# apache/brpc

Measured on NVIDIA H100. Metric: echo QPS, 1 KB baidu_std, higher is better.
Workload: dtype u8

## Files before the change

### brpc_b200/abi.py

```python
import atexit
import ctypes as C
import gc
import os

import numpy as np

_HERE = os.path.dirname(os.path.abspath(__file__))
lib_path = os.environ.get("B2RPC_LIB") or os.path.join(_HERE, "libb2rpc.so")

B2_OK, B2_E_INVAL, B2_E_NO_DEVICE, B2_E_CUDA, B2_E_CAPACITY, B2_E_NOMEM = 0, -1, -2, -3, -4, -5

RUN_DT = np.dtype([("socket_id", "<u8"), ("offset", "<u4"), ("length", "<u4"),
                   ("preferred_proto", "<i4"), ("flags", "<u4")])
RUN_STATUS_DT = np.dtype([("consumed", "<u4"), ("parse_error", "<u4"), ("n_msgs", "<u4"), ("first_msg", "<u4"),
                          ("preferred_proto", "<i4"), ("n_unanswered", "<u4"), ("resp_off", "<u4"), ("resp_bytes", "<u4")])
H2_FRAME_DT = np.dtype([("type", "u1"), ("flags", "u1"), ("pad", "<u2"), ("stream_id", "<u4"), ("payload_off", "<u4"), ("payload_len", "<u4")])
HPACK_BLOCK_DT = np.dtype([("conn", "<u4"), ("offset", "<u4"), ("length", "<u4"), ("reserved", "<u4")])
H2_RUN_STATUS_DT = np.dtype([("consumed", "<u4"), ("parse_error", "<u4"), ("n_msgs", "<u4"), ("first_msg", "<u4"), ("ctrl_off", "<u4"), ("ctrl_len", "<u4"),
                             ("remote_max_frame_size", "<u4"), ("remote_stream_window_size", "<u4")])
REQUEST_DT = np.dtype([("kind", "<u4"), ("flags", "<u4"), ("method_idx", "<i4"), ("timeout_ms", "<i4"), ("correlation_id", "<i8"), ("log_id", "<i8"),
                       ("compress_type", "<i4"), ("checksum_type", "<i4"), ("frame_type", "<i4"), ("payload_off", "<u4"), ("payload_len", "<u4"),
                       ("attachment_off", "<u4"), ("attachment_len", "<u4"), ("reserved", "<u4")])
REPLY_DT = np.dtype([("flags", "<u4"), ("error_code", "<i4"), ("correlation_id", "<i8"), ("compress_type", "<i4"), ("checksum_type", "<i4"),
                     ("content_type", "<i4"), ("error_text_off", "<u4"), ("error_text_len", "<u4"), ("body_off", "<u4"), ("body_len", "<u4"),
                     ("attachment_off", "<u4"), ("attachment_len", "<u4"), ("checksum_value_off", "<u4"), ("checksum_value_len", "<u4"),
                     ("extra_streams_off", "<u4"), ("n_extra_streams", "<u4"), ("user_fields_off", "<u4"), ("n_user_fields", "<u4"),
                     ("reserved", "<u4"), ("stream_id", "<i8")])
H2_RESPONSE_DT = np.dtype([("conn", "<u4"), ("stream_id", "<u4"), ("status_code", "<i4"), ("flags", "<u4"), ("content_type_off", "<u4"),
                           ("content_type_len", "<u4"), ("body_off", "<u4"), ("body_len", "<u4"), ("grpc_status", "<i4"),
                           ("grpc_message_off", "<u4"), ("grpc_message_len", "<u4"), ("reserved", "<u4")])
H2_REQUEST_DT = np.dtype([("conn", "<u4"), ("flags", "<u4"), ("path_off", "<u4"), ("path_len", "<u4"), ("authority_off", "<u4"),
                          ("authority_len", "<u4"), ("content_type_off", "<u4"), ("content_type_len", "<u4"), ("body_off", "<u4"),
                          ("body_len", "<u4"), ("extra_off", "<u4"), ("extra_len", "<u4")])
H2_PEER_UPDATE_DT = np.dtype([("set", "<u4"), ("header_table_size", "<u4"), ("max_frame_size", "<u4"), ("stream_window_size", "<u4"), ("conn_window_add", "<i8")])
H2_REQUEST_RESULT_DT = np.dtype([("status", "<i4"), ("stream_id", "<u4"), ("out_off", "<u4"), ("out_len", "<u4")])
H2_MSG_DT = np.dtype([("run_idx", "<u4"), ("stream_id", "<u4"), ("headers_off", "<u4"), ("headers_len", "<u4"), ("n_headers", "<u4"),
                      ("body_off", "<u4"), ("body_len", "<u4"), ("http_method", "<u4"), ("content_type", "<u4"), ("flags", "<u4"),
                      ("method_idx", "<i4"), ("msg_off", "<u4"), ("msg_len", "<u4"), ("path_off", "<u4"), ("path_len", "<u4"), ("reserved", "<u4")])
H2_CALL_DT = np.dtype([("run_idx", "<u4"), ("stream_id", "<u4"), ("how", "<u4"), ("status_code", "<i4"), ("error_code", "<i4"), ("grpc_status", "<i4"),
                       ("headers_off", "<u4"), ("headers_len", "<u4"), ("n_headers", "<u4"), ("body_off", "<u4"), ("body_len", "<u4"),
                       ("msg_off", "<u4"), ("msg_len", "<u4"), ("error_off", "<u4"), ("error_len", "<u4"), ("flags", "<u4")])
H2_FLAG_GUNZIPPED, H2_FLAG_GUNZIP_HOST, H2_FLAG_NO_GRPC_ENCODING = 64, 128, 256
H2_FLAG_ANSWERED = 512
H2_REPLY_SPAN_DT = np.dtype([("off", "<u4"), ("len", "<u4"), ("n_answered", "<u4"), ("reserved", "<u4")])
MSG_DT = np.dtype([("run_idx", "<u4"), ("frame_off", "<u4"), ("body_size", "<u4"), ("meta_size", "<u4"),
                   ("correlation_id", "<i8"), ("log_id", "<i8"),
                   ("attachment_size", "<i4"), ("compress_type", "<i4"), ("checksum_type", "<i4"), ("error_code", "<i4"),
                   ("has_bits", "<u2"), ("protocol", "u1"), ("content_type", "u1"),
                   ("method_idx", "<i2"), ("status", "<u2"), ("resp_off", "<u4"), ("resp_len", "<u4")])
assert RUN_DT.itemsize == 24 and RUN_STATUS_DT.itemsize == 32 and MSG_DT.itemsize == 64
STREAM_DESC_DT = np.dtype([("stream_id", "<i8"), ("remote_stream_id", "<i8"), ("host_socket_id", "<u8"), ("flags", "<u4"), ("max_buf_size", "<u4")])
STREAM_MSG_DT = np.dtype([("stream_id", "<i8"), ("first_frame", "<u4"), ("n_frames", "<u4"), ("off", "<u4"), ("len", "<u4"), ("flags", "<u4"), ("reserved", "<u4")])
STREAM_EVENT_DT = np.dtype([("stream_id", "<i8"), ("host_socket_id", "<u8"), ("local_consumed", "<u8"), ("remote_consumed", "<u8"), ("n_msgs", "<u4"),
                            ("first_msg", "<u4"), ("consumed_bytes", "<u4"), ("flags", "<u4"), ("fb_off", "<u4"), ("fb_len", "<u4"), ("close_off", "<u4"),
                            ("close_len", "<u4"), ("handover_msg", "<u4"), ("pending_bytes", "<u4"), ("reserved", "<u4", (2,))])
assert STREAM_DESC_DT.itemsize == 32 and STREAM_MSG_DT.itemsize == 32 and STREAM_EVENT_DT.itemsize == 80
STREAM_CONNECTED, STREAM_NEED_FEEDBACK, STREAM_CLOSED, STREAM_HANDED_OVER = 1, 2, 4, 8
STREAM_MSG_IN_INPUT = 1
STREAM_EV_REMOTE_CONSUMED_MOVED, STREAM_EV_CLOSED_BY_RST, STREAM_EV_CLOSED_BY_CLOSE, STREAM_EV_HANDED_OVER, STREAM_EV_WRITABLE = 1, 2, 4, 8, 16
STREAM_WRITE_DT = np.dtype([("stream_id", "<i8"), ("flags", "<u4"), ("src_off", "<u4"), ("src_len", "<u4"), ("reserved", "<u4")])
STREAM_WRITE_RESULT_DT = np.dtype([("status", "<i4"), ("n_frames", "<u4"), ("out_off", "<u4"), ("out_len", "<u4"), ("produced", "<u8"),
                                   ("host_socket_id", "<u8")])
assert STREAM_WRITE_DT.itemsize == 24 and STREAM_WRITE_RESULT_DT.itemsize == 32
STREAM_W_FROM_MSG = 1
STREAM_W_NOT_CONNECTED, STREAM_W_HANDED_OVER = -1, -2
STREAM_W_DEFAULT_SEGMENT = 512 << 20


class Method(C.Structure):
    _fields_ = [("service_full_name", C.c_char_p), ("service_name", C.c_char_p), ("method_name", C.c_char_p),
                ("request_type_name", C.c_char_p), ("handler", C.c_int32), ("echo_attachment", C.c_int32),
                ("response_checksum_type", C.c_int32), ("response_compress_type", C.c_int32)]


class Options(C.Structure):
    _fields_ = [("device", C.c_int32), ("max_batch_bytes", C.c_uint32), ("max_msgs", C.c_uint32),
                ("max_runs", C.c_uint32), ("max_resp_bytes", C.c_uint32), ("tile_bytes", C.c_uint32),
                ("max_body_size", C.c_uint64)]


class BatchResult(C.Structure):
    _fields_ = [("runs", C.c_void_p), ("n_runs", C.c_uint32),
                ("msgs", C.c_void_p), ("n_msgs", C.c_uint32),
                ("resp", C.c_void_p), ("resp_bytes", C.c_uint32),
                ("kernel_ms", C.c_float), ("n_launches", C.c_uint32), ("refs", C.c_void_p), ("iov", C.c_void_p)]


class H2RingResult(C.Structure):
    _fields_ = [("runs", C.c_void_p), ("n_runs", C.c_uint32), ("n_msgs", C.c_uint32), ("msgs", C.c_void_p), ("out", C.c_void_p),
                ("region", C.c_uint32), ("replies", C.c_void_p), ("spans", C.c_void_p), ("status", C.c_int32)]


assert C.sizeof(H2RingResult) == 64


class H2ClientRingResult(C.Structure):
    _fields_ = [("runs", C.c_void_p), ("n_runs", C.c_uint32), ("n_calls", C.c_uint32), ("calls", C.c_void_p), ("out", C.c_void_p),
                ("region", C.c_uint32), ("n_reqs", C.c_uint32), ("reqs", C.c_void_p), ("req_out", C.c_void_p), ("status", C.c_int32),
                ("reserved", C.c_uint32)]


assert C.sizeof(H2ClientRingResult) == 64


class StreamState(C.Structure):
    _fields_ = [("local_consumed", C.c_uint64), ("remote_consumed", C.c_uint64), ("pending_bytes", C.c_uint32), ("flags", C.c_uint32),
                ("error_code", C.c_int32), ("reserved", C.c_uint32)]


class StreamBatchResult(C.Structure):
    _fields_ = [("msgs", C.c_void_p), ("n_msgs", C.c_uint32), ("events", C.c_void_p), ("n_events", C.c_uint32),
                ("out", C.c_void_p), ("out_bytes", C.c_uint32), ("ctrl", C.c_void_p), ("ctrl_bytes", C.c_uint32),
                ("run_ctrl", C.c_void_p), ("n_runs", C.c_uint32)]


REF_DT = np.dtype([("prefix_len", "<u4"), ("src_off", "<u4"), ("src_len", "<u4"), ("reserved", "<u4")])
IOVEC_DT = np.dtype([("base", "<u8"), ("len", "<u8")])
INPUT_COPY, INPUT_PULL, RESP_COPY, RESP_BY_REF, RESP_IOVEC = 0, 1, 0, 1, 2


class ResidentKernel(C.Structure):
    _fields_ = [("name", C.c_char_p), ("regs", C.c_uint32), ("threads", C.c_uint32), ("smem_bytes", C.c_uint32), ("fits", C.c_uint32)]


class B2Error(RuntimeError):
    def __init__(self, code, text):
        super().__init__("b2rpc error %d: %s" % (code, text))
        self.code = code


def _load():
    if not os.path.exists(lib_path):
        raise ImportError("brpc_b200/libb2rpc.so is missing: run `python -c 'import __graft_entry__ as g; g.build()'` "
                          "(nvcc, sm_90a).  There is no CPU fallback.")
    l = C.CDLL(lib_path)
    l.b2_last_error.restype = C.c_char_p
    l.b2_version.restype = C.c_char_p
    l.b2_ctx_create.argtypes = [C.POINTER(Options), C.POINTER(C.c_void_p)]
    l.b2_ctx_destroy.argtypes = [C.c_void_p]
    l.b2_register_method.argtypes = [C.c_void_p, C.POINTER(Method)]
    l.b2_set_server_identity.argtypes = [C.c_void_p, C.c_char_p]
    l.b2_set_stream_handler.argtypes = [C.c_void_p, C.c_int]
    l.b2_set_protocols.argtypes = [C.c_void_p, C.c_uint32]
    l.b2_block_alloc.restype = C.c_void_p; l.b2_block_alloc.argtypes = [C.c_size_t]
    l.b2_block_free.argtypes = [C.c_void_p]
    l.b2_block_pool_host_allocs.restype = C.c_uint64
    l.b2_set_modes.argtypes = [C.c_void_p, C.c_int, C.c_int]
    l.b2_ring_start.argtypes = [C.c_void_p]; l.b2_ring_stop.argtypes = [C.c_void_p]
    l.b2_ring_submit.argtypes = [C.c_void_p, C.c_void_p, C.c_uint32, C.c_void_p, C.c_uint32, C.POINTER(C.c_uint32)]
    l.b2_ring_wait.argtypes = [C.c_void_p, C.c_uint32, C.POINTER(BatchResult)]
    l.b2_ring_launches.restype = C.c_uint64; l.b2_ring_launches.argtypes = [C.c_void_p]
    l.b2_ring_phase_ns.argtypes = [C.c_void_p, C.c_uint32, C.c_void_p]
    l.b2_latency_probe.argtypes = [C.c_void_p, C.c_void_p, C.c_uint32, C.c_void_p, C.c_uint32, C.c_uint32, C.c_int, C.c_void_p]
    l.b2_process_batch.argtypes = [C.c_void_p, C.c_void_p, C.c_uint32, C.c_void_p, C.c_uint32, C.POINTER(BatchResult)]
    l.b2_batch_submit.argtypes = [C.c_void_p, C.c_void_p, C.c_uint32, C.c_void_p, C.c_uint32]
    l.b2_batch_collect.argtypes = [C.c_void_p, C.POINTER(BatchResult)]
    l.b2_batch_upload.argtypes = [C.c_void_p, C.c_void_p, C.c_uint32, C.c_void_p, C.c_uint32]
    l.b2_batch_execute.argtypes = [C.c_void_p, C.POINTER(C.c_float), C.POINTER(C.c_uint32)]
    l.b2_batch_execute_many.argtypes = [C.c_void_p, C.c_uint32, C.POINTER(C.c_float), C.POINTER(C.c_uint32)]
    l.b2_batch_launch.argtypes = [C.c_void_p]
    l.b2_batch_wait.argtypes = [C.c_void_p]
    l.b2_elapsed_ms.argtypes = [C.c_void_p, C.c_void_p, C.POINTER(C.c_float)]
    l.b2_batch_download.argtypes = [C.c_void_p, C.POINTER(BatchResult)]
    l.b2_batch_info.argtypes = [C.c_void_p, C.c_void_p]
    l.b2_resident_plan.argtypes = [C.c_void_p, C.POINTER(ResidentKernel), C.c_int]
    l.b2_device_pci_bus_id.argtypes = [C.c_int, C.c_char_p, C.c_int]
    l.b2_stage_times.argtypes = [C.c_void_p, C.POINTER(C.c_char_p), C.POINTER(C.c_float), C.c_int]
    l.b2_crc32c_batch.argtypes = [C.c_void_p, C.c_void_p, C.c_uint32, C.c_void_p, C.c_void_p, C.c_uint32, C.c_void_p]
    l.b2_snappy_uncompress_batch.argtypes = [C.c_void_p, C.c_void_p, C.c_uint32, C.c_void_p, C.c_void_p, C.c_uint32,
                                             C.c_void_p, C.c_uint32, C.c_void_p, C.c_void_p]
    l.b2_snappy_compress_batch.argtypes = [C.c_void_p, C.c_void_p, C.c_uint32, C.c_void_p, C.c_void_p, C.c_uint32,
                                           C.c_void_p, C.c_uint32, C.c_void_p, C.c_void_p]
    l.b2_crc32c_extend.restype = C.c_uint32; l.b2_crc32c_extend.argtypes = [C.c_uint32, C.c_char_p, C.c_size_t]
    l.b2_snappy_max_compressed_length.restype = C.c_size_t; l.b2_snappy_max_compressed_length.argtypes = [C.c_size_t]
    l.b2_snappy_raw_compress.argtypes = [C.c_char_p, C.c_size_t, C.c_void_p, C.POINTER(C.c_size_t)]
    l.b2_snappy_get_uncompressed_length.argtypes = [C.c_char_p, C.c_size_t, C.POINTER(C.c_size_t)]
    l.b2_snappy_raw_uncompress.argtypes = [C.c_char_p, C.c_size_t, C.c_void_p]
    l.b2_hpack_reset.argtypes = [C.c_void_p, C.c_uint32, C.c_uint32]
    l.b2_hpack_decode_batch.argtypes = [C.c_void_p, C.c_void_p, C.c_uint32, C.c_void_p, C.c_uint32, C.c_void_p, C.c_uint32,
                                        C.c_void_p, C.c_void_p, C.c_void_p]
    l.b2_h2_scan_batch.argtypes = [C.c_void_p, C.c_void_p, C.c_uint32, C.c_void_p, C.c_uint32, C.c_uint32, C.c_void_p, C.c_uint32,
                                   C.c_void_p, C.c_void_p, C.c_void_p]
    l.b2_h2_conn_reset.argtypes = [C.c_void_p, C.c_uint32]
    l.b2_h2_configure.argtypes = [C.c_void_p, C.c_uint32, C.c_uint32, C.c_uint32]
    l.b2_h2_process_batch.argtypes = [C.c_void_p, C.c_void_p, C.c_uint32, C.c_void_p, C.c_uint32, C.c_void_p, C.c_void_p, C.c_uint32,
                                      C.POINTER(C.c_uint32), C.c_void_p, C.c_uint32]
    l.b2_h2_pack_requests.argtypes = [C.c_void_p, C.c_void_p, C.c_uint32, C.c_void_p, C.c_uint32, C.c_void_p, C.c_uint32, C.c_void_p]
    l.b2_h2_conn_set_next_stream_id.argtypes = [C.c_void_p, C.c_uint32, C.c_uint32]
    l.b2_h2_conn_peer_update.argtypes = [C.c_void_p, C.c_uint32, C.c_void_p]
    l.b2_h2_client_conn_reset.argtypes = [C.c_void_p, C.c_uint32]
    l.b2_h2_client_process_batch.argtypes = [C.c_void_p, C.c_void_p, C.c_uint32, C.c_void_p, C.c_uint32, C.c_void_p, C.c_void_p, C.c_uint32,
                                             C.POINTER(C.c_uint32), C.c_void_p, C.c_uint32]
    l.b2_h2_client_abandon_streams.argtypes = [C.c_void_p, C.c_uint32, C.c_void_p, C.c_uint32]
    l.b2_h2_conn_set_gunzip.argtypes = [C.c_void_p, C.c_uint32, C.c_int]
    l.b2_h2_serve_batch.argtypes = [C.c_void_p, C.c_void_p, C.c_uint32, C.c_void_p, C.c_uint32, C.c_void_p, C.c_void_p, C.c_uint32,
                                    C.POINTER(C.c_uint32), C.c_void_p, C.c_uint32, C.c_void_p, C.c_uint32, C.c_void_p]
    l.b2_h2_ring_enable.argtypes = [C.c_void_p, C.c_uint32, C.c_uint32, C.c_uint32, C.c_uint32]
    l.b2_h2_ring_submit.argtypes = [C.c_void_p, C.c_void_p, C.c_uint32, C.c_void_p, C.c_uint32, C.POINTER(C.c_uint32)]
    l.b2_h2_ring_wait.argtypes = [C.c_void_p, C.c_uint32, C.POINTER(H2RingResult)]
    l.b2_h2_client_ring_enable.argtypes = [C.c_void_p, C.c_uint32, C.c_uint32, C.c_uint32, C.c_uint32, C.c_uint32]
    l.b2_h2_client_ring_submit.argtypes = [C.c_void_p, C.c_void_p, C.c_uint32, C.c_void_p, C.c_uint32, C.c_void_p, C.c_uint32, C.POINTER(C.c_uint32)]
    l.b2_h2_client_ring_wait.argtypes = [C.c_void_p, C.c_uint32, C.POINTER(H2ClientRingResult)]
    l.b2_h2_pack_responses.argtypes = [C.c_void_p, C.c_void_p, C.c_uint32, C.c_void_p, C.c_uint32, C.c_void_p, C.c_uint32, C.c_void_p, C.c_void_p]
    l.b2_pack_requests.argtypes = [C.c_void_p, C.c_void_p, C.c_uint32, C.c_void_p, C.c_uint32, C.c_void_p, C.c_uint32, C.c_void_p, C.c_void_p]
    l.b2_pack_responses.argtypes = [C.c_void_p, C.c_void_p, C.c_uint32, C.c_void_p, C.c_uint32, C.c_void_p, C.c_uint32, C.c_void_p, C.c_void_p]
    l.b2_stream_configure.argtypes = [C.c_void_p, C.c_uint32, C.c_uint32, C.c_uint32]
    l.b2_stream_open.argtypes = [C.c_void_p, C.c_void_p, C.c_uint32]
    l.b2_stream_set_connected.argtypes = [C.c_void_p, C.c_int64, C.c_int64, C.c_uint32, C.c_void_p, C.c_uint32, C.POINTER(C.c_uint32)]
    l.b2_stream_close.argtypes = [C.c_void_p, C.c_int64, C.c_void_p, C.c_uint32, C.POINTER(C.c_uint32)]
    l.b2_stream_query.argtypes = [C.c_void_p, C.c_int64, C.POINTER(StreamState)]
    l.b2_stream_take_pending.argtypes = [C.c_void_p, C.c_int64, C.c_void_p, C.c_uint32, C.POINTER(C.c_uint32)]
    l.b2_stream_results.argtypes = [C.c_void_p, C.POINTER(StreamBatchResult)]
    l.b2_stream_ring_enable.argtypes = [C.c_void_p, C.c_uint32]
    l.b2_stream_write.argtypes = [C.c_void_p, C.c_void_p, C.c_uint32, C.c_void_p, C.c_uint32, C.c_uint32, C.c_void_p, C.c_uint32, C.c_void_p]
    l.b2_counters_read.argtypes = [C.c_void_p, C.POINTER(C.c_int64)]
    l.b2_counters_device_ptr.restype = C.c_void_p; l.b2_counters_device_ptr.argtypes = [C.c_void_p]
    return l


lib = _load()

ABI_SYMBOLS = ["b2_ctx_create", "b2_ctx_destroy", "b2_last_error", "b2_version", "b2_register_method",
               "b2_set_server_identity", "b2_set_stream_handler", "b2_set_protocols", "b2_block_alloc", "b2_block_free", "b2_block_pool_host_allocs", "b2_set_modes", "b2_ring_start", "b2_ring_stop", "b2_ring_submit", "b2_ring_wait", "b2_ring_launches", "b2_ring_phase_ns", "b2_latency_probe", "b2_process_batch", "b2_batch_submit", "b2_batch_collect", "b2_batch_upload",
               "b2_batch_execute", "b2_batch_execute_many", "b2_batch_download", "b2_batch_launch", "b2_batch_wait",
               "b2_elapsed_ms", "b2_batch_info", "b2_resident_plan", "b2_device_pci_bus_id", "b2_stage_times", "b2_crc32c_batch", "b2_crc32c_extend", "b2_snappy_max_compressed_length", "b2_snappy_raw_compress", "b2_snappy_get_uncompressed_length", "b2_snappy_raw_uncompress", "b2_snappy_uncompress_batch", "b2_snappy_compress_batch", "b2_hpack_reset", "b2_hpack_decode_batch", "b2_pack_requests", "b2_pack_responses", "b2_h2_scan_batch", "b2_h2_conn_reset", "b2_h2_configure", "b2_h2_process_batch", "b2_h2_pack_responses", "b2_counters_read",
               "b2_counters_device_ptr", "b2_counters_allreduce", "b2_h2_pack_requests", "b2_h2_conn_set_next_stream_id", "b2_h2_conn_peer_update",
               "b2_h2_client_conn_reset", "b2_h2_client_process_batch", "b2_h2_client_abandon_streams", "b2_h2_conn_set_gunzip",
               "b2_h2_serve_batch", "b2_stream_configure", "b2_stream_open", "b2_stream_set_connected", "b2_stream_close", "b2_stream_query",
               "b2_stream_take_pending", "b2_stream_results", "b2_stream_write", "b2_stream_ring_enable", "b2_h2_ring_enable", "b2_h2_ring_submit",
               "b2_h2_ring_wait", "b2_h2_client_ring_enable", "b2_h2_client_ring_submit", "b2_h2_client_ring_wait"]

ECHO_METHOD = dict(service_full_name=b"example.EchoService", service_name=b"EchoService", method_name=b"Echo",
                   request_type_name=b"example.EchoRequest", handler=1, echo_attachment=1,
                   response_checksum_type=0, response_compress_type=0)


def _check(rc):
    if rc < 0:
        raise B2Error(rc, (lib.b2_last_error() or b"").decode("utf-8", "replace"))
    return rc


def _view(ptr, nbytes, dtype=np.uint8):
    return np.ctypeslib.as_array((C.c_uint8 * nbytes).from_address(ptr)).view(dtype) if nbytes else np.zeros(0, dtype)


_in_gc = [False]
_reclaimed = []


def _gc_phase(phase, info):
    _in_gc[0] = phase == "start"


def _destroy_reclaimed():
    hs = _reclaimed[:]
    del _reclaimed[:]
    for h in hs:
        lib.b2_ring_stop(h)
    for h in hs:
        lib.b2_ctx_destroy(h)


gc.callbacks.append(_gc_phase)
atexit.register(_destroy_reclaimed)


class PinnedBuffer:

    def __init__(self, nbytes):
        self.ptr = lib.b2_block_alloc(nbytes)
        if not self.ptr:
            raise B2Error(B2_E_NOMEM, "b2_block_alloc failed")
        self.nbytes = nbytes
        self.array = np.ctypeslib.as_array((C.c_uint8 * nbytes).from_address(self.ptr))

    def free(self):
        if self.ptr:
            lib.b2_block_free(self.ptr)
            self.ptr = None

    def __del__(self):
        try:
            self.free()
        except Exception:
            pass


class Context:

    def __init__(self, device=0, max_batch_bytes=64 << 20, max_msgs=1 << 20, max_runs=4096, max_resp_bytes=0,
                 tile_bytes=0, max_body_size=0, methods=(ECHO_METHOD,), server_identity=None, stream_handler=0):
        _destroy_reclaimed()
        opt = Options(device, max_batch_bytes, max_msgs, max_runs, max_resp_bytes, tile_bytes, max_body_size)
        h = C.c_void_p()
        _check(lib.b2_ctx_create(C.byref(opt), C.byref(h)))
        self._h = h
        self._keep = []
        for m in methods:
            self.register_method(**m)
        if server_identity:
            _check(lib.b2_set_server_identity(self._h, server_identity))
        if stream_handler:
            _check(lib.b2_set_stream_handler(self._h, stream_handler))

    def close(self):
        if getattr(self, "_h", None):
            lib.b2_ctx_destroy(self._h)
            self._h = None
        _destroy_reclaimed()

    def __del__(self):
        try:
            if _in_gc[0] and getattr(self, "_h", None):
                _reclaimed.append(self._h)
                self._h = None
            else:
                self.close()
        except Exception:
            pass

    def register_method(self, **kw):
        m = Method(**kw)
        self._keep.append(m)
        return _check(lib.b2_register_method(self._h, C.byref(m)))

    @staticmethod
    def _views(res):
        runs = np.ctypeslib.as_array((C.c_uint8 * (32 * res.n_runs)).from_address(res.runs)).view(RUN_STATUS_DT) \
            if res.n_runs else np.zeros(0, RUN_STATUS_DT)
        msgs = np.ctypeslib.as_array((C.c_uint8 * (64 * res.n_msgs)).from_address(res.msgs)).view(MSG_DT) \
            if res.n_msgs else np.zeros(0, MSG_DT)
        resp = np.ctypeslib.as_array((C.c_uint8 * res.resp_bytes).from_address(res.resp)) \
            if res.resp_bytes else np.zeros(0, np.uint8)
        return runs, msgs, resp

    @staticmethod
    def _info(res):
        refs = None
        if res.refs and res.n_msgs:
            refs = np.ctypeslib.as_array((C.c_uint8 * (16 * res.n_msgs)).from_address(res.refs)).view(REF_DT)
        iov = None
        if res.iov and res.n_msgs:
            iov = np.ctypeslib.as_array((C.c_uint8 * (32 * res.n_msgs)).from_address(res.iov)).view(IOVEC_DT)
        return {"kernel_ms": res.kernel_ms, "n_launches": res.n_launches, "refs": refs, "iov": iov}

    def _ring_bytes(self, data, ptr, nbytes):
        if ptr is None:
            data = np.ascontiguousarray(data, dtype=np.uint8); ptr, nbytes = data.ctypes.data, data.nbytes
            self._ring_keep = data
        return ptr, nbytes

    def ring_start(self):
        _check(lib.b2_ring_start(self._h))

    def ring_stop(self):
        _check(lib.b2_ring_stop(self._h))

    def ring_submit(self, data, runs, ptr=None, nbytes=None):
        runs = np.ascontiguousarray(runs, dtype=RUN_DT)
        ptr, nbytes = self._ring_bytes(data, ptr, nbytes)
        t = C.c_uint32(0)
        _check(lib.b2_ring_submit(self._h, ptr, nbytes, runs.ctypes.data, len(runs), C.byref(t)))
        return t.value

    def ring_wait(self, ticket):
        res = BatchResult()
        _check(lib.b2_ring_wait(self._h, ticket, C.byref(res)))
        rs, msgs, resp = self._views(res)
        return rs, msgs, resp, self._info(res)

    def latency_probe(self, ptr, nbytes, runs, iters, use_ring):
        runs = np.ascontiguousarray(runs, dtype=RUN_DT)
        us = np.zeros(iters, np.float32)
        _check(lib.b2_latency_probe(self._h, ptr, nbytes, runs.ctypes.data, len(runs), iters, 1 if use_ring else 0, us.ctypes.data))
        return us

    def ring_phase_ns(self, ticket):
        out = (C.c_uint64 * 4)()
        _check(lib.b2_ring_phase_ns(self._h, ticket, out))
        return list(out)

    def ring_launches(self):
        return int(lib.b2_ring_launches(self._h))

    def set_protocols(self, mask):
        _check(lib.b2_set_protocols(self._h, mask))

    def set_modes(self, input_mode=INPUT_COPY, resp_mode=RESP_COPY):
        _check(lib.b2_set_modes(self._h, input_mode, resp_mode))

    def process_batch(self, data, runs):
        data = np.ascontiguousarray(data, dtype=np.uint8)
        runs = np.ascontiguousarray(runs, dtype=RUN_DT)
        res = BatchResult()
        _check(lib.b2_process_batch(self._h, data.ctypes.data, data.nbytes, runs.ctypes.data, len(runs), C.byref(res)))
        rs, msgs, resp = self._views(res)
        return rs, msgs, resp, self._info(res)

    def upload(self, data, runs):
        data = np.ascontiguousarray(data, dtype=np.uint8)
        runs = np.ascontiguousarray(runs, dtype=RUN_DT)
        _check(lib.b2_batch_upload(self._h, data.ctypes.data, data.nbytes, runs.ctypes.data, len(runs)))

    def upload_ptr(self, ptr, nbytes, runs):
        runs = np.ascontiguousarray(runs, dtype=RUN_DT)
        _check(lib.b2_batch_upload(self._h, ptr, nbytes, runs.ctypes.data, len(runs)))

    def execute(self):
        ms, n = C.c_float(0), C.c_uint32(0)
        _check(lib.b2_batch_execute(self._h, C.byref(ms), C.byref(n)))
        return ms.value, n.value

    def execute_many(self, steps):
        ms, n = C.c_float(0), C.c_uint32(0)
        _check(lib.b2_batch_execute_many(self._h, steps, C.byref(ms), C.byref(n)))
        return ms.value, n.value

    def launch(self):
        _check(lib.b2_batch_launch(self._h))

    def wait(self):
        _check(lib.b2_batch_wait(self._h))

    def elapsed_ms_to(self, other):
        ms = C.c_float(0)
        _check(lib.b2_elapsed_ms(self._h, other._h, C.byref(ms)))
        return ms.value

    def download(self):
        res = BatchResult()
        _check(lib.b2_batch_download(self._h, C.byref(res)))
        rs, msgs, resp = self._views(res)
        return rs, msgs, resp, self._info(res)

    def process_batch_ptr(self, ptr, nbytes, runs):
        runs = np.ascontiguousarray(runs, dtype=RUN_DT)
        res = BatchResult()
        _check(lib.b2_process_batch(self._h, ptr, nbytes, runs.ctypes.data, len(runs), C.byref(res)))
        rs, msgs, resp = self._views(res)
        return rs, msgs, resp, self._info(res)

    def submit_ptr(self, ptr, nbytes, runs):
        runs = np.ascontiguousarray(runs, dtype=RUN_DT)
        self._submitted_runs = runs
        _check(lib.b2_batch_submit(self._h, ptr, nbytes, runs.ctypes.data, len(runs)))

    def collect(self):
        res = BatchResult()
        _check(lib.b2_batch_collect(self._h, C.byref(res)))
        rs, msgs, resp = self._views(res)
        return rs, msgs, resp, self._info(res)

    def stream_configure(self, max_streams, pending_bytes, out_bytes=0):
        _check(lib.b2_stream_configure(self._h, max_streams, pending_bytes, out_bytes))

    def stream_open(self, streams):
        if not isinstance(streams, np.ndarray):
            a = np.zeros(len(streams), STREAM_DESC_DT)
            for i, t in enumerate(streams):
                a[i] = tuple(t) + (0,) * (5 - len(t))
            streams = a
        streams = np.ascontiguousarray(streams, dtype=STREAM_DESC_DT)
        _check(lib.b2_stream_open(self._h, streams.ctypes.data, len(streams)))

    def stream_set_connected(self, stream_id, remote_stream_id, flags=0):
        buf = C.create_string_buffer(64); n = C.c_uint32(0)
        _check(lib.b2_stream_set_connected(self._h, stream_id, remote_stream_id, flags, buf, 64, C.byref(n)))
        return buf.raw[:n.value]

    def stream_close(self, stream_id):
        buf = C.create_string_buffer(64); n = C.c_uint32(0)
        _check(lib.b2_stream_close(self._h, stream_id, buf, 64, C.byref(n)))
        return buf.raw[:n.value]

    def stream_query(self, stream_id):
        st = StreamState()
        _check(lib.b2_stream_query(self._h, stream_id, C.byref(st)))
        return {"local_consumed": st.local_consumed, "remote_consumed": st.remote_consumed, "pending_bytes": st.pending_bytes,
                "flags": st.flags, "error_code": st.error_code}

    def stream_take_pending(self, stream_id, cap):
        buf = np.zeros(max(1, cap), np.uint8); n = C.c_uint32(0)
        _check(lib.b2_stream_take_pending(self._h, stream_id, buf.ctypes.data, cap, C.byref(n)))
        return buf[:n.value].tobytes()

    def stream_ring_enable(self, out_bytes):
        _check(lib.b2_stream_ring_enable(self._h, out_bytes))

    def stream_results(self):
        r = StreamBatchResult()
        _check(lib.b2_stream_results(self._h, C.byref(r)))
        return (_view(r.msgs, 32 * r.n_msgs, STREAM_MSG_DT), _view(r.events, 80 * r.n_events, STREAM_EVENT_DT), _view(r.out, r.out_bytes, np.uint8),
                _view(r.ctrl, r.ctrl_bytes, np.uint8), _view(r.run_ctrl, 8 * r.n_runs, np.uint32).reshape(-1, 2))

    def stream_write(self, writes, data=None, max_segment_size=0, out_cap=None, out=None):
        if not isinstance(writes, np.ndarray):
            a = np.zeros(len(writes), STREAM_WRITE_DT)
            for i, t in enumerate(writes):
                a[i] = tuple(t) + (0,) * (5 - len(t))
            writes = a
        writes = np.ascontiguousarray(writes, dtype=STREAM_WRITE_DT)
        n = len(writes)
        if data is None:
            ptr, nb = None, 0
        else:
            data = np.ascontiguousarray(np.frombuffer(data, np.uint8) if isinstance(data, (bytes, bytearray)) else data, dtype=np.uint8)
            ptr, nb = data.ctypes.data, data.nbytes
        if out is None:
            if out_cap is None:
                seg = max_segment_size or STREAM_W_DEFAULT_SEGMENT
                lens = np.where(writes["flags"] & STREAM_W_FROM_MSG, 0, writes["src_len"]).astype(np.int64)
                if np.any(writes["flags"] & STREAM_W_FROM_MSG):
                    sm = self.stream_results()[0]
                    fm = (writes["flags"] & STREAM_W_FROM_MSG) != 0
                    idx = writes["src_off"][fm].astype(np.int64)
                    lens[fm] = np.where(idx < len(sm), sm["len"][np.minimum(idx, max(len(sm) - 1, 0))] if len(sm) else 0, 0)
                nfr = np.maximum(1, (lens + seg - 1) // seg)
                out_cap = int(((lens + nfr * 38 + 15) // 16 * 16).sum())
            out = np.empty(max(1, out_cap), np.uint8)
        res = np.zeros(n, STREAM_WRITE_RESULT_DT)
        _check(lib.b2_stream_write(self._h, ptr, nb, writes.ctypes.data, n, max_segment_size, out.ctypes.data, out.nbytes, res.ctypes.data))
        return res, out

    def batch_info(self):
        out = (C.c_uint32 * 4)()
        _check(lib.b2_batch_info(self._h, out))
        return {"tile_bytes": out[0], "n_tiles": out[1], "spec_k": out[2], "fused": bool(out[3])}

    def resident_plan(self):
        out = (ResidentKernel * 8)()
        n = _check(lib.b2_resident_plan(self._h, out, 8))
        return [{"name": out[i].name.decode(), "regs": out[i].regs, "threads": out[i].threads, "smem_bytes": out[i].smem_bytes,
                 "fits": out[i].fits} for i in range(min(n, 8))]

    def stage_times(self):
        names = (C.c_char_p * 16)()
        ms = (C.c_float * 16)()
        n = lib.b2_stage_times(self._h, names, ms, 16)
        return [(names[i].decode(), ms[i]) for i in range(max(0, min(n, 16)))]
# ... 216 lines not shown
```

### brpc_b200/csrc/b2_api.cu

```cuda
#include <cuda_runtime.h>
#include <dlfcn.h>
#include <stdio.h>
#include <time.h>
#include <stdlib.h>
#include <string.h>
#include <algorithm>
#include <mutex>
#include <string>
#include <unordered_map>
#include <vector>
#include "b2_kernels.cuh"
#include "b2_h2.cuh"

using namespace b2;

static thread_local char g_err[512] = "";
static void set_err(const char* fmt, const char* a = "", const char* b = "") { snprintf(g_err, sizeof g_err, fmt, a, b); }

#define CU(call)                                                                          \
    do {                                                                                  \
        cudaError_t e_ = (call);                                                          \
        if (e_ != cudaSuccess) { set_err("%s: %s", #call, cudaGetErrorString(e_)); return B2_E_CUDA; } \
    } while (0)

namespace {
constexpr int kMaxStages = 16;
constexpr uint32_t kSmallBytes = 128 << 10;
constexpr uint32_t kSmallRuns = 512, kSmallMsgs = 1024;
constexpr size_t kSmallBlock = 64 + kSmallRuns * 32 + kSmallMsgs * (64 + 16) + (kSmallBytes + kSmallMsgs * 80 + 4096);
struct SmallLayout { uint32_t msgs, resp, off_rs, off_msgs, off_refs, off_resp, total; };
SmallLayout small_layout(uint32_t nbytes, uint32_t n_runs, uint32_t max_msgs) {
    const uint32_t mb = std::min(std::min(nbytes / 12 + 1, kSmallMsgs), max_msgs), resp = nbytes + mb * 80 + 2048, off_msgs = 64 + n_runs * 32;
    const uint32_t off_refs = off_msgs + mb * 64, off_resp = (off_refs + mb * 16 + 255u) & ~255u;
    return { mb, resp, 64, off_msgs, off_refs, off_resp, off_resp + resp };
}
constexpr uint32_t kSecEvents = 64, kSecMsgs = kSecEvents + kSmallMsgs * 80, kSecCtrl = kSecMsgs + kSmallMsgs * 32,
                   kSecRunCtrl = kSecCtrl + 3 * kStreamCtrlMax * kSmallMsgs, kSecOut = kSecRunCtrl + kSmallRuns * 8;
struct Stage { const char* name; cudaEvent_t ev; };
enum class RingKind { none, batch, batch_streams, h2_server, h2_client };
struct SlotLayout {
    uint64_t end = 256;
    uint32_t add(uint64_t bytes) { const uint64_t off = end; end = (end + bytes + 255u) & ~255ull; return (uint32_t)off; }
};
}

enum : int { kPlanFused, kPlanSearch, kPlanWalk, kPlanResolve, kPlanSlow, kPlanKernels };
struct b2_ctx {
    b2_options opt;
    DevConfig cfg;
    std::vector<DevMethod> methods;
    uint8_t* d_bytes = nullptr; b2_run* d_runs = nullptr; uint32_t* d_run_tile_base = nullptr;
    TileRec* d_tiles = nullptr; uint32_t* d_tile_base = nullptr; uint32_t* d_tile_scratch = nullptr; uint32_t* d_tile_spec = nullptr; b2_run_status* d_run_status = nullptr;
    uint32_t* d_frame_off = nullptr; uint32_t* d_frame_run = nullptr; b2_msg_desc* d_msgs = nullptr; MsgAux* d_aux = nullptr; PackJob* d_jobs = nullptr; uint32_t* d_slow_idx = nullptr; uint8_t* d_heads = nullptr;
    uint32_t* d_slot = nullptr; uint32_t* d_scan_tmp = nullptr; uint8_t* d_resp = nullptr; uint8_t* d_unz = nullptr; uint16_t* d_snappy_tab = nullptr; HpackState* d_hpack = nullptr; H2Conn* d_h2 = nullptr; H2Stream* d_h2_streams = nullptr; uint8_t* d_h2_slots = nullptr; uint32_t h2_max_conns = B2_H2_MAX_CONNS, h2_pending = B2_H2_MAX_PENDING, h2_stream_bytes = B2_H2_STREAM_BYTES; uint64_t h2_last_in = 0, h2_last_out = 0;
    uint32_t* d_frame_row = nullptr; uint4* d_rows = nullptr;
    std::vector<uint8_t> h2_gunzip; uint8_t* d_h2_gz_merge = nullptr;
    RingKind ring_kind = RingKind::none; RingDev ring_dev = {}; H2RingDev h2r_dev = {}; H2ClientRingDev h2c_dev = {};
    uint8_t* ring_slots = nullptr; volatile uint32_t* ring_ctl = nullptr; uint32_t* d_ring_ticket = nullptr; cudaStream_t ring_stream = nullptr;
    uint32_t ring_next = 1, ring_stride = 0; bool ring_collected[8] = { true, true, true, true, true, true, true, true };
    const void* ring_bytes[8] = {}; const void* ring_pin_base = nullptr; unsigned long long ring_pin_dev = 0; uint64_t ring_launches = 0;
    StreamPass sp_ring = {}; uint8_t* d_st_ring = nullptr; uint32_t ring_next_wait = 1, st_view_ticket = 0;
    uint32_t h2r_max_bytes = 0, h2r_msg_cap = 0, h2r_out_cap = 0, h2r_replies_cap = 0;
    uint32_t h2c_max_bytes = 0, h2c_call_cap = 0, h2c_out_cap = 0, h2c_max_reqs = 0, h2c_req_out_cap = 0;
    ulonglong2* d_iov = nullptr; b2_iovec* h_iov = nullptr; const void* host_bytes = nullptr;
    uint4* d_refs = nullptr; b2_resp_ref* h_refs = nullptr; int input_mode = B2_INPUT_COPY, resp_mode = B2_RESP_COPY; const uint8_t* pull_bytes = nullptr;
    uint32_t* d_crc_adv = nullptr; unsigned long long* d_counters = nullptr; uint32_t* d_totals = nullptr; DevMethod* d_methods = nullptr;
    size_t meta_tile_off = 0; uint32_t max_tiles = 0; uint32_t n_sms = 132; bool use_tma_pack = true; uint32_t stage_mask = 7;
    StreamPass sp = {}; bool has_streams = false, stream_armed = false, stream_ran = false, stream_valid = false;
    uint32_t st_max = 0, st_open = 0; std::vector<long long> st_keys; std::vector<uint8_t> st_state; std::vector<uint32_t> st_pool, st_pool_free;
    void* d_st_block[10] = {}; void* h_st_mapped[5] = {}; uint32_t* h_st_cnts = nullptr; uint8_t* h_st_out = nullptr; uint8_t* h_st_ctl = nullptr; uint8_t* d_st_ctl = nullptr;
    b2_stream_msg* h_st_msgs = nullptr; b2_stream_event* h_st_events = nullptr; uint8_t* h_st_ctrl = nullptr; uint32_t* h_st_run_ctrl = nullptr;
    cudaEvent_t st_ev[6] = {};
    const uint8_t* st_input = nullptr;
    void* d_sw[4] = {}; size_t sw_have[4] = {}; SwRec* h_sw_recs = nullptr; size_t h_sw_have = 0; uint32_t* h_sw_cnts = nullptr;
    cudaEvent_t sw_ev[8] = {}; bool sw_ran = false;
    b2_run_status* h_run_status = nullptr; b2_msg_desc* h_msgs = nullptr; uint8_t* h_resp = nullptr;
    uint32_t* h_totals = nullptr; uint32_t* h_run_tile_base = nullptr;
    uint32_t n_runs = 0, n_tiles = 0, nbytes = 0, max_run_tiles = 0; uint64_t covered = 0;
    bool uploaded = false, executed = false;
    cudaStream_t stream = nullptr;
    cudaEvent_t ev[kMaxStages + 1];
    const char* stage_names[kMaxStages];
    int n_stages = 0;
    float last_kernel_ms = 0.f; uint32_t last_launches = 0;
    cudaEvent_t ev_first = nullptr, ev_last = nullptr; bool first_pending = true;
    bool profile_stages = false; bool allow_small = true; bool use_fused = true; bool fused_last = false; bool slow_heavy = false;
    bool adaptive_tile = false; bool dense = false; uint32_t avg_frame = 0;
    uint8_t* d_meta = nullptr; uint8_t* h_meta = nullptr;
    uint8_t* d_small = nullptr; uint8_t* h_small = nullptr;
    bool small = false, small_copy_queued = false, use_fused_small = true; SmallLayout sm = {};
    b2_resident_kernel plan[kPlanKernels] = {}; uint32_t sm_regs = 0, sm_smem = 0, sm_warps = 0, sm_blocks = 0, block_smem_reserve = 0;
};

enum : unsigned { kDevInput = 1, kDevBatch = 2 };
static void overwrites(b2_ctx* c, unsigned what) {
    if (what & kDevInput) { c->h2_last_in = 0; c->h2_last_out = 0; if (c->st_input == c->d_bytes) c->st_input = nullptr; }
    if (what & kDevBatch) { c->uploaded = false; c->executed = false; }
}

static uint32_t g_crc_tab_host[256];
static void crc_table_init() {
    for (uint32_t i = 0; i < 256; i++) {
        uint32_t c = i;
        for (int k = 0; k < 8; k++) c = (c & 1) ? (c >> 1) ^ 0x82f63b78u : (c >> 1);
        g_crc_tab_host[i] = c;
    }
}

extern "C" const char* b2_last_error(void) { return g_err; }
extern "C" const char* b2_version(void) { return "brpc_b200 0.1 (sm_90a)"; }

namespace {
struct BlockPool {
    std::mutex mu;
    static constexpr size_t kSmall = 8192, kSlab = 4u << 20;
    std::vector<uint8_t*> slabs; std::vector<void*> small_free;
    std::unordered_map<void*, int> large_class;
    std::vector<void*> large_free[40];
    uint64_t n_host_alloc = 0;
    void* alloc(size_t size) {
        std::lock_guard<std::mutex> g(mu);
        if (size <= kSmall) {
            if (small_free.empty()) {
                uint8_t* slab = nullptr;
                if (cudaHostAlloc((void**)&slab, kSlab, cudaHostAllocMapped | cudaHostAllocPortable) != cudaSuccess) return nullptr;
                n_host_alloc++; slabs.push_back(slab);
                for (size_t o = 0; o + kSmall <= kSlab; o += kSmall) small_free.push_back(slab + o);
            }
            void* p = small_free.back(); small_free.pop_back(); return p;
        }
        int cls = 14; while (((size_t)1 << cls) < size) cls++;
        if (cls >= 40) return nullptr;
        if (!large_free[cls].empty()) { void* p = large_free[cls].back(); large_free[cls].pop_back(); return p; }
        void* p = nullptr;
        if (cudaHostAlloc(&p, ((size_t)1 << cls) + 1024, cudaHostAllocMapped | cudaHostAllocPortable) != cudaSuccess) return nullptr;
        n_host_alloc++; large_class[p] = cls;
        return p;
    }
    void free(void* p) {
        std::lock_guard<std::mutex> g(mu);
        auto it = large_class.find(p);
        if (it != large_class.end()) { large_free[it->second].push_back(p); return; }
        small_free.push_back(p);
    }
};
BlockPool& block_pool() { static BlockPool* p = new BlockPool; return *p; }
}
extern "C" void* b2_block_alloc(size_t size) {
    void* p = block_pool().alloc(size ? size : 1);
    if (!p) set_err("cudaHostAlloc failed");
    return p;
}
extern "C" void b2_block_free(void* p) { if (p) block_pool().free(p); }
extern "C" uint64_t b2_block_pool_host_allocs(void) { std::lock_guard<std::mutex> g(block_pool().mu); return block_pool().n_host_alloc; }

static void ring_halt(b2_ctx* c);
static void stream_free(b2_ctx* c);
static bool ring_busy(const b2_ctx* c) { for (uint32_t k = 0; k < kRingSlots; k++) if (!c->ring_collected[k]) return true; return false; }
static uint8_t* ring_slot(const b2_ctx* c, uint32_t ticket) { return c->ring_slots + (size_t)(ticket % kRingSlots) * c->ring_stride; }
static bool h2_ring_refuses(b2_ctx* c, bool writes_h2_state) {
    if (c->ring_kind != RingKind::h2_server && c->ring_kind != RingKind::h2_client) return false;
    if (ring_busy(c)) { set_err(c->ring_kind == RingKind::h2_server ? "an h2 ring ticket is outstanding: b2_h2_ring_wait it first" : "an h2 client ring ticket is outstanding: b2_h2_client_ring_wait it first"); return true; }
    if (writes_h2_state) ring_halt(c);
    return false;
}
extern "C" void b2_ctx_destroy(b2_ctx* c) {
    if (!c) return;
    cudaSetDevice(c->opt.device);
    ring_halt(c);
    if (c->ring_stream) cudaStreamDestroy(c->ring_stream);
    if (c->ring_slots) cudaFreeHost(c->ring_slots);
    if (c->ring_ctl) cudaFreeHost((void*)c->ring_ctl);
    cudaFree(c->d_ring_ticket);
    cudaFree(c->d_bytes); cudaFree(c->d_runs); cudaFree(c->d_run_tile_base); cudaFree(c->d_tiles); cudaFree(c->d_tile_base); cudaFree(c->d_tile_scratch); cudaFree(c->d_tile_spec);
    cudaFree(c->d_run_status); cudaFree(c->d_frame_off); cudaFree(c->d_frame_run); cudaFree(c->d_msgs); cudaFree(c->d_aux); cudaFree(c->d_jobs); cudaFree(c->d_slow_idx); cudaFree(c->d_heads); cudaFree(c->d_slot);
    cudaFree(c->d_scan_tmp); cudaFree(c->d_resp); cudaFree(c->d_unz); cudaFree(c->d_snappy_tab); cudaFree(c->d_refs); cudaFree(c->d_iov); cudaFreeHost(c->h_iov); cudaFree(c->d_frame_row); cudaFree(c->d_rows); cudaFreeHost(c->h_refs); cudaFree(c->d_hpack); cudaFree(c->d_h2); cudaFree(c->d_h2_streams); cudaFree(c->d_h2_slots); cudaFree(c->d_h2_gz_merge); cudaFree(c->d_counters); cudaFree(c->d_totals); cudaFree(c->d_methods); cudaFree(c->d_crc_adv); cudaFree(c->d_meta); cudaFree(c->d_small); cudaFreeHost(c->h_meta); cudaFreeHost(c->h_small);
    cudaFreeHost(c->h_run_status); cudaFreeHost(c->h_msgs); cudaFreeHost(c->h_resp); cudaFreeHost(c->h_totals);
    cudaFreeHost(c->h_run_tile_base);
    stream_free(c);
    for (int i = 0; i <= kMaxStages; i++) if (c->ev[i]) cudaEventDestroy(c->ev[i]);
    if (c->stream) cudaStreamDestroy(c->stream);
    delete c;
}

extern "C" int b2_ctx_create(const b2_options* o, b2_ctx** out) {
    if (!o || !out) { set_err("null argument"); return B2_E_INVAL; }
    int ndev = 0;
    if (cudaGetDeviceCount(&ndev) != cudaSuccess || ndev == 0) {
        set_err("no CUDA device: brpc_b200 has no CPU path"); return B2_E_NO_DEVICE;
    }
    if (o->device < 0 || o->device >= ndev) { set_err("bad device ordinal"); return B2_E_INVAL; }
    if (o->max_batch_bytes == 0 || o->max_batch_bytes >= (1u << 31) || o->max_msgs == 0 || o->max_runs == 0) {
        set_err("capacities must be non-zero and max_batch_bytes < 2 GiB"); return B2_E_INVAL;
    }
    CU(cudaSetDevice(o->device));
    b2_ctx* c = new b2_ctx();
    { int v = 132; cudaDeviceGetAttribute(&v, cudaDevAttrMultiProcessorCount, o->device); c->n_sms = (uint32_t)v; }
    for (int i = 0; i <= kMaxStages; i++) c->ev[i] = nullptr;
    c->opt = *o;
    c->adaptive_tile = o->tile_bytes == 0;
    uint32_t tile = o->tile_bytes ? o->tile_bytes : 8192;
    if (tile < 512 || (tile & (tile - 1))) { delete c; set_err("tile_bytes must be a power of two >= 512"); return B2_E_INVAL; }
    c->opt.tile_bytes = tile;
    if (c->opt.max_resp_bytes == 0) {
        uint64_t r = (uint64_t)o->max_batch_bytes + (uint64_t)o->max_msgs * 64 + (1u << 20);
        c->opt.max_resp_bytes = r > 0xfffffff0ull ? 0xfffffff0u : (uint32_t)r;
    }
    memset(&c->cfg, 0, sizeof c->cfg);
    c->cfg.max_body_size = o->max_body_size ? o->max_body_size : (64ull << 20);
    c->cfg.proto_mask = kProtoMaskDefault;
    c->cfg.tile_bytes = tile;
    c->cfg.tile_shift = 0; while ((1u << c->cfg.tile_shift) < tile) c->cfg.tile_shift++;
    c->max_tiles = o->max_batch_bytes / tile + o->max_runs + 1;
    const uint32_t scan_blocks = o->max_msgs / (kScanBlock * kScanItems) + 2;
#define ALLOC(ptr, bytes) do { if (cudaMalloc((void**)&(ptr), (bytes)) != cudaSuccess) { set_err("cudaMalloc %s failed", #ptr); b2_ctx_destroy(c); return B2_E_NOMEM; } } while (0)
#define HALLOC(ptr, bytes) do { if (cudaHostAlloc((void**)&(ptr), (bytes), cudaHostAllocDefault) != cudaSuccess) { set_err("cudaHostAlloc %s failed", #ptr); b2_ctx_destroy(c); return B2_E_NOMEM; } } while (0)
    ALLOC(c->d_bytes, (size_t)o->max_batch_bytes + 1024);
    ALLOC(c->d_runs, sizeof(b2_run) * (size_t)o->max_runs);
    ALLOC(c->d_run_tile_base, 4 * ((size_t)o->max_runs + 1));
    ALLOC(c->d_tiles, sizeof(TileRec) * (size_t)c->max_tiles);
    ALLOC(c->d_tile_base, 4 * (size_t)c->max_tiles);
    ALLOC(c->d_tile_scratch, 12 * (size_t)c->max_tiles);
    {
        size_t dense_tiles = (size_t)o->max_batch_bytes / 2048 + o->max_runs + 1; if (dense_tiles > c->max_tiles) dense_tiles = c->max_tiles;
        size_t words = (size_t)kSpecK * c->max_tiles; if ((size_t)kSpecKDense * dense_tiles > words) words = (size_t)kSpecKDense * dense_tiles;
        ALLOC(c->d_tile_spec, 4 * words);
    }
    ALLOC(c->d_run_status, sizeof(b2_run_status) * (size_t)o->max_runs);
    ALLOC(c->d_frame_off, 4 * (size_t)o->max_msgs);
    ALLOC(c->d_frame_run, 4 * (size_t)o->max_msgs);
    ALLOC(c->d_msgs, sizeof(b2_msg_desc) * (size_t)o->max_msgs);
    ALLOC(c->d_aux, sizeof(MsgAux) * (size_t)o->max_msgs);
    ALLOC(c->d_jobs, sizeof(PackJob) * (size_t)o->max_msgs);
    ALLOC(c->d_refs, sizeof(uint4) * (size_t)o->max_msgs);
    ALLOC(c->d_slow_idx, sizeof(uint32_t) * (size_t)o->max_msgs);
    ALLOC(c->d_heads, (size_t)kHeadBytes * (size_t)o->max_msgs);
    ALLOC(c->d_slot, 4 * ((size_t)o->max_msgs + 1));
    ALLOC(c->d_scan_tmp, 4 * (size_t)scan_blocks);
    ALLOC(c->d_resp, (size_t)c->opt.max_resp_bytes + 1024);
    ALLOC(c->d_unz, 2 * (size_t)c->opt.max_resp_bytes + 1024);
    ALLOC(c->d_snappy_tab, (size_t)kSnappyWarps * kSnappyMaxTable * 2);
    ALLOC(c->d_hpack, sizeof(HpackState) * (size_t)B2_HPACK_MAX_CONNS);
    CU(cudaMemset(c->d_hpack, 0, sizeof(HpackState) * (size_t)B2_HPACK_MAX_CONNS));
    ALLOC(c->d_counters, 8 * B2_N_COUNTERS);
    ALLOC(c->d_totals, 64);
    ALLOC(c->d_methods, sizeof(DevMethod) * 64);
    ALLOC(c->d_crc_adv, (kCrcHotWords + kCrcTreeWords) * 4);
    ALLOC(c->d_meta, (size_t)o->max_runs * 28 + 16 * (size_t)c->max_tiles + 64);
    ALLOC(c->d_small, kSmallBlock);
    HALLOC(c->h_meta, (size_t)o->max_runs * 28 + 16 * (size_t)c->max_tiles + 64);
    HALLOC(c->h_small, kSmallBlock);
    HALLOC(c->h_run_status, sizeof(b2_run_status) * (size_t)o->max_runs);
    HALLOC(c->h_msgs, sizeof(b2_msg_desc) * (size_t)o->max_msgs);
    HALLOC(c->h_refs, sizeof(b2_resp_ref) * (size_t)o->max_msgs);
    HALLOC(c->h_resp, (size_t)c->opt.max_resp_bytes);
    HALLOC(c->h_totals, 64);
    HALLOC(c->h_run_tile_base, 4 * ((size_t)o->max_runs + 1));
    CU(cudaMemset(c->d_counters, 0, 8 * B2_N_COUNTERS));
    CU(cudaMemset(c->d_bytes, 0, (size_t)o->max_batch_bytes + 1024));
    CU(cudaStreamCreateWithFlags(&c->stream, cudaStreamNonBlocking));
    for (int i = 0; i <= kMaxStages; i++) CU(cudaEventCreate(&c->ev[i]));
    CU(cudaEventCreate(&c->ev_first)); CU(cudaEventCreate(&c->ev_last));
    crc_table_init();
    CU(cudaMemcpyToSymbol(c_crc_table, g_crc_tab_host, sizeof g_crc_tab_host));
    {
        std::vector<uint32_t> tab(kCrcHotWords + kCrcTreeWords);
        auto adv = [&](uint32_t x, int bytes) { for (int k = 0; k < bytes; k++) x = g_crc_tab_host[x & 0xff] ^ (x >> 8); return x; };
        for (int k = 0; k < 16; k++) for (uint32_t b = 0; b < 256; b++) tab[k * 256 + b] = adv(g_crc_tab_host[b], k);
        for (int j = 0; j < 4; j++) for (uint32_t b = 0; b < 256; b++) tab[(16 + j) * 256 + b] = adv(b << (8 * j), 512);
        for (int t = 0; t < 5; t++) for (int j = 0; j < 4; j++) for (uint32_t b = 0; b < 256; b++)
            tab[kCrcHotWords + (t * 4 + j) * 256 + b] = adv(b << (8 * j), 16 << t);
        CU(cudaMemcpy(c->d_crc_adv, tab.data(), tab.size() * 4, cudaMemcpyHostToDevice));
    }
    CU(cudaFuncSetAttribute(k_resolve, cudaFuncAttributeMaxDynamicSharedMemorySize, 200 * 1024));
    CU(cudaFuncSetAttribute(k_pack_slow<false>, cudaFuncAttributeMaxDynamicSharedMemorySize, (int)(8 * kSnapRing)));
    CU(cudaFuncSetAttribute(k_pack_tma<kPackGroup>, cudaFuncAttributeMaxDynamicSharedMemorySize, (int)(sizeof(PackWarpSmem) * kPackWarps)));
    CU(cudaFuncSetAttribute(k_pack_tma<kPackGroupSmall>, cudaFuncAttributeMaxDynamicSharedMemorySize, (int)(sizeof(PackWarpSmem) * kPackWarps)));
    if (const char* e = getenv("B2_PACK")) c->use_tma_pack = strcmp(e, "reg") != 0;
    if (const char* e = getenv("B2_SMALL")) c->use_fused_small = strcmp(e, "off") != 0;
    if (const char* e = getenv("B2_FUSED")) c->use_fused = strcmp(e, "off") != 0;
    CU(cudaFuncSetAttribute(k_fused, cudaFuncAttributeMaxDynamicSharedMemorySize, (int)(sizeof(FusedWarpSmem) * (kFusedWarps > kFusedWarpsDense ? kFusedWarps : kFusedWarpsDense))));
    CU(cudaFuncSetAttribute(k_small, cudaFuncAttributeMaxDynamicSharedMemorySize, (int)sizeof(SmallSmem)));
#if defined(__NVCC__)
    {
        const void* fn[kPlanKernels] = { (const void*)k_fused, (const void*)k_tile_search, (const void*)k_tile_walk, (const void*)k_resolve, (const void*)k_pack_slow<true> };
        const char* name[kPlanKernels] = { "k_fused", "k_tile_search", "k_tile_walk", "k_resolve", "k_pack_slow<true>" };
        const uint32_t threads[kPlanKernels] = { 0, kSearchThreadsFused, 128, 256, kSlowLiteThreads };
        for (int k = 0; k < kPlanKernels; k++) {
            cudaFuncAttributes a;
            CU(cudaFuncGetAttributes(&a, fn[k]));
            c->plan[k].name = name[k]; c->plan[k].regs = (uint32_t)a.numRegs; c->plan[k].threads = threads[k]; c->plan[k].smem_bytes = (uint32_t)a.sharedSizeBytes;
        }
        int v[5] = {};
        CU(cudaDeviceGetAttribute(&v[0], cudaDevAttrMaxRegistersPerMultiprocessor, o->device));
        CU(cudaDeviceGetAttribute(&v[1], cudaDevAttrMaxSharedMemoryPerMultiprocessor, o->device));
        CU(cudaDeviceGetAttribute(&v[2], cudaDevAttrMaxThreadsPerMultiProcessor, o->device));
        CU(cudaDeviceGetAttribute(&v[3], cudaDevAttrMaxBlocksPerMultiprocessor, o->device));
        CU(cudaDeviceGetAttribute(&v[4], cudaDevAttrReservedSharedMemoryPerBlock, o->device));
        c->sm_regs = (uint32_t)v[0]; c->sm_smem = (uint32_t)v[1]; c->sm_warps = (uint32_t)v[2] / 32; c->sm_blocks = (uint32_t)v[3]; c->block_smem_reserve = (uint32_t)v[4];
    }
#endif
    *out = c;
    return B2_OK;
}

extern "C" int b2_set_server_identity(b2_ctx* c, const char* ip_port) {
    if (!c) return B2_E_INVAL;
    if (h2_ring_refuses(c, true)) return B2_E_INVAL;
    const size_t n = ip_port ? strlen(ip_port) : 0;
    if (n >= sizeof c->cfg.identity) { set_err("identity too long"); return B2_E_INVAL; }
    memset(c->cfg.identity, 0, sizeof c->cfg.identity);
    if (n) memcpy(c->cfg.identity, ip_port, n);
    c->cfg.identity_len = (uint32_t)n;
    return B2_OK;
}

extern "C" int b2_set_modes(b2_ctx* c, int input_mode, int resp_mode) {
    if (!c || (input_mode != B2_INPUT_COPY && input_mode != B2_INPUT_PULL) || (resp_mode != B2_RESP_COPY && resp_mode != B2_RESP_BY_REF && resp_mode != B2_RESP_IOVEC)) { set_err("bad mode"); return B2_E_INVAL; }
    static_assert(sizeof(b2_resp_ref) == sizeof(uint4), "b2_resp_ref is 16 bytes");
    static_assert(sizeof(b2_iovec) == sizeof(ulonglong2) && sizeof(void*) == 8, "b2_iovec is a 16-byte struct iovec");
    if (resp_mode == B2_RESP_IOVEC && !c->d_iov) {
        CU(cudaSetDevice(c->opt.device));
        if (cudaMalloc((void**)&c->d_iov, 32 * (size_t)c->opt.max_msgs) != cudaSuccess || cudaHostAlloc((void**)&c->h_iov, 32 * (size_t)c->opt.max_msgs, cudaHostAllocDefault) != cudaSuccess) {
            cudaFree(c->d_iov); c->d_iov = nullptr; cudaGetLastError(); set_err("allocation of the iovec list failed"); return B2_E_NOMEM;
        }
    }
    if (input_mode == B2_INPUT_PULL && !c->d_rows) {
        CU(cudaSetDevice(c->opt.device));
        const uint32_t tile = c->adaptive_tile ? 32768u : c->opt.tile_bytes;
        const size_t tiles = (size_t)c->opt.max_batch_bytes / tile + c->opt.max_runs + 1;
        const size_t rows = tiles * (tile >= 2048 ? kSpecKDense : kSpecK);
        if (cudaMalloc((void**)&c->d_rows, rows * 128) != cudaSuccess || cudaMalloc((void**)&c->d_frame_row, 4 * (size_t)c->opt.max_msgs) != cudaSuccess) {
            cudaFree(c->d_rows); c->d_rows = nullptr; cudaGetLastError(); set_err("cudaMalloc of the pull-mode row stash failed"); return B2_E_NOMEM;
        }
    }
    ring_halt(c);
    c->input_mode = input_mode; c->resp_mode = resp_mode; c->cfg.by_ref = resp_mode != B2_RESP_COPY; c->cfg.pull = input_mode == B2_INPUT_PULL; c->cfg.pull_vecs = resp_mode != B2_RESP_COPY ? 6u : 8u;
    overwrites(c, kDevBatch);
    return B2_OK;
}

extern "C" int b2_set_protocols(b2_ctx* c, uint32_t mask) {
    const uint32_t known = (1u << 1) | (1u << 2) | (1u << 3) | (1u << 4) | (1u << 12);
    if (!c || mask == 0 || (mask & ~known)) { set_err("unknown protocol in mask (baidu_std 1, streaming_rpc 2, hulu_pbrpc 3, sofa_pbrpc 4, nshead 12)"); return B2_E_INVAL; }
    ring_halt(c);
    c->cfg.proto_mask = mask;
    return B2_OK;
}

extern "C" int b2_set_stream_handler(b2_ctx* c, int kind) {
    if (!c || (kind != B2_STREAM_DESC_ONLY && kind != B2_STREAM_SNAPPY_UNCOMPRESS)) { set_err("bad stream handler"); return B2_E_INVAL; }
    c->cfg.stream_handler = (uint32_t)kind;
    return B2_OK;
}

extern "C" int b2_register_method(b2_ctx* c, const b2_method* m) {
    if (!c || !m || !m->service_full_name || !m->service_name || !m->method_name || !m->request_type_name) { set_err("null argument"); return B2_E_INVAL; }
    if (c->methods.size() >= 64) { set_err("method table full"); return B2_E_CAPACITY; }
    DevMethod d; memset(&d, 0, sizeof d);
    std::string full = std::string(m->service_full_name) + "." + m->method_name;
    if (full.size() >= sizeof d.full_method || strlen(m->service_name) >= sizeof d.service_short ||
        strlen(m->service_full_name) >= sizeof d.service_full || strlen(m->request_type_name) >= sizeof d.request_type) {
        set_err("method names too long"); return B2_E_INVAL;
    }
    memcpy(d.full_method, full.data(), full.size()); d.full_method_len = (uint32_t)full.size();
    d.service_short_len = (uint32_t)strlen(m->service_name); memcpy(d.service_short, m->service_name, d.service_short_len);
    d.service_full_len = (uint32_t)strlen(m->service_full_name); memcpy(d.service_full, m->service_full_name, d.service_full_len);
    d.request_type_len = (uint32_t)strlen(m->request_type_name); memcpy(d.request_type, m->request_type_name, d.request_type_len);
    d.handler = m->handler; d.echo_attachment = m->echo_attachment;
    d.response_checksum_type = m->response_checksum_type; d.response_compress_type = m->response_compress_type;
    ring_halt(c);
    c->methods.push_back(d);
    c->cfg.n_methods = (uint32_t)c->methods.size();
    CU(cudaSetDevice(c->opt.device));
    CU(cudaMemcpy(c->d_methods, c->methods.data(), sizeof(DevMethod) * c->methods.size(), cudaMemcpyHostToDevice));
    return (int)c->methods.size() - 1;
}

static BatchPtrs make_ptrs(b2_ctx* c) {
    BatchPtrs B;
    B.bytes = c->d_bytes; B.runs = c->d_runs; B.run_tile_base = c->d_run_tile_base; B.tiles = c->d_tiles;
    B.tile_base = c->d_tile_base; B.tile_scratch = c->d_tile_scratch; B.tile_spec = c->d_tile_spec; B.run_status = c->d_run_status; B.frame_off = c->d_frame_off; B.frame_run = c->d_frame_run; B.frame_row = c->d_frame_row; B.rows = c->d_rows; B.msgs = c->d_msgs;
    B.aux = c->d_aux; B.jobs = c->d_jobs; B.refs = c->d_refs; B.slow_idx = c->d_slow_idx; B.heads = c->d_heads; B.slot = c->d_slot; B.scan_tmp = c->d_scan_tmp; B.resp = c->d_resp; B.unz = c->d_unz; B.snappy_tab = c->d_snappy_tab; B.counters = c->d_counters;
    B.totals = c->d_totals; B.methods = c->d_methods; B.crc_adv = c->d_crc_adv;
    B.n_runs = c->n_runs; B.n_tiles = c->n_tiles; B.max_msgs = c->opt.max_msgs; B.max_resp = c->opt.max_resp_bytes;
    B.runs = reinterpret_cast<const b2_run*>(c->d_meta);
    B.run_tile_base = reinterpret_cast<const uint32_t*>(c->d_meta + (size_t)c->n_runs * sizeof(b2_run));
    B.tile_info = reinterpret_cast<const uint4*>(c->d_meta + c->meta_tile_off);
    if (c->input_mode == B2_INPUT_PULL) B.bytes = c->pull_bytes;
    if (c->small) {
        B.refs = reinterpret_cast<uint4*>(c->d_small + c->sm.off_refs);
        B.totals = reinterpret_cast<uint32_t*>(c->d_small);
        B.run_status = reinterpret_cast<b2_run_status*>(c->d_small + c->sm.off_rs);
        B.msgs = reinterpret_cast<b2_msg_desc*>(c->d_small + c->sm.off_msgs);
        B.resp = c->d_small + c->sm.off_resp;
        B.max_msgs = c->sm.msgs; B.max_resp = c->sm.resp;
    }
    return B;
}

extern "C" int b2_batch_upload(b2_ctx* c, const void* bytes, uint32_t nbytes, const b2_run* runs, uint32_t n_runs) {
    if (!c || (!bytes && nbytes) || (!runs && n_runs)) { set_err("null argument"); return B2_E_INVAL; }
    if (h2_ring_refuses(c, false)) return B2_E_INVAL;
    if ((c->input_mode != B2_INPUT_PULL && nbytes > c->opt.max_batch_bytes) || nbytes >= (1u << 31) || n_runs > c->opt.max_runs) { set_err("batch exceeds ctx capacity"); return B2_E_CAPACITY; }
    uint64_t covered = 0; for (uint32_t r = 0; r < n_runs; r++) covered += runs[r].length;
    if (c->input_mode == B2_INPUT_PULL && covered > c->opt.max_batch_bytes) { set_err("runs exceed ctx capacity"); return B2_E_CAPACITY; }
    c->stream_valid = false; c->st_view_ticket = 0;
    c->covered = covered;
    CU(cudaSetDevice(c->opt.device));
    if (!c->avg_frame && n_runs && runs[0].length >= 12 && (uint64_t)runs[0].offset + 12 <= nbytes) {
        const uint8_t* f = static_cast<const uint8_t*>(bytes) + runs[0].offset;
        uint32_t w[2]; memcpy(w, f, 8);
        const uint32_t body = __builtin_bswap32(w[1]);
        if ((w[0] == kMagicPRPC || w[0] == kMagicSTRM) && body <= c->cfg.max_body_size && body < (1u << 30)) c->avg_frame = 12 + body;
    }
    if (c->adaptive_tile) {
        uint32_t t = 8192;
        const uint32_t per_tile = c->input_mode == B2_INPUT_PULL ? 48u : 6u;
        if (c->input_mode == B2_INPUT_PULL && t < 32768) t = 32768;
        while (t < (1u << 20) && t < per_tile * c->avg_frame) t <<= 1;
        c->cfg.tile_bytes = t; c->cfg.tile_shift = 0; while ((1u << c->cfg.tile_shift) < t) c->cfg.tile_shift++;
    }
    const uint32_t shift = c->cfg.tile_shift, tile = c->cfg.tile_bytes;
    c->dense = tile >= 2048 && c->avg_frame && (uint64_t)c->avg_frame * kSpecK < tile;
    c->cfg.spec_k = c->dense ? kSpecKDense : kSpecK;
    uint64_t nt = 0; uint32_t max_rt = 0;
    for (uint32_t r = 0; r < n_runs; r++) {
        if ((runs[r].offset & 15u) || (uint64_t)runs[r].offset + runs[r].length > nbytes) { set_err("run offset must be 16-aligned and inside the batch"); return B2_E_INVAL; }
        c->h_run_tile_base[r] = (uint32_t)nt;
        const uint32_t t = (uint32_t)(((uint64_t)runs[r].length + tile - 1) >> shift);
        nt += t; if (t > max_rt) max_rt = t;
    }
    c->h_run_tile_base[n_runs] = (uint32_t)nt;
    if (nt > c->max_tiles) { set_err("too many tiles"); return B2_E_CAPACITY; }
    c->n_runs = n_runs; c->n_tiles = (uint32_t)nt; c->nbytes = nbytes; c->max_run_tiles = max_rt; c->host_bytes = bytes;
    const size_t tile_off = ((size_t)n_runs * sizeof(b2_run) + 4 * ((size_t)n_runs + 1) + 15) & ~(size_t)15;
    const size_t meta_bytes = tile_off + 16 * (size_t)nt;
    c->meta_tile_off = tile_off;
    if (n_runs) memcpy(c->h_meta, runs, (size_t)n_runs * sizeof(b2_run));
    memcpy(c->h_meta + (size_t)n_runs * sizeof(b2_run), c->h_run_tile_base, 4 * ((size_t)n_runs + 1));
    {
        uint32_t* ti = reinterpret_cast<uint32_t*>(c->h_meta + tile_off);
        for (uint32_t r = 0; r < n_runs; r++) {
            const uint32_t t0 = c->h_run_tile_base[r], t1 = c->h_run_tile_base[r + 1];
            for (uint32_t t = t0; t < t1; t++) { uint32_t* q = ti + 4 * (size_t)t; q[0] = runs[r].offset; q[1] = runs[r].length; q[2] = t - t0; q[3] = r | (runs[r].flags << 24); }
        }
    }
    overwrites(c, kDevInput | kDevBatch);
    if (c->input_mode == B2_INPUT_PULL) {
        void* dp = nullptr;
        if (nbytes && cudaHostGetDevicePointer(&dp, const_cast<void*>(bytes), 0) != cudaSuccess) {
            cudaGetLastError(); set_err("B2_INPUT_PULL: bytes must be pinned + mapped memory from b2_block_alloc"); return B2_E_INVAL;
        }
        c->pull_bytes = static_cast<const uint8_t*>(dp);
    } else if (nbytes) CU(cudaMemcpyAsync(c->d_bytes, bytes, nbytes, cudaMemcpyHostToDevice, c->stream));
    CU(cudaMemcpyAsync(c->d_meta, c->h_meta, meta_bytes, cudaMemcpyHostToDevice, c->stream));
    c->small = c->allow_small && nbytes <= kSmallBytes && n_runs <= kSmallRuns && n_runs > 0;
    if (c->small) c->sm = small_layout(nbytes, n_runs, c->opt.max_msgs);
    if (const char* e = getenv("B2_STAGE_MASK")) c->stage_mask = (uint32_t)atoi(e);
    c->uploaded = true;
    return B2_OK;
}

static const char* const kStreamStages[5] = { "stream_route", "stream_alloc", "stream_group", "stream_run", "stream_rst" };
static uint32_t grid(uint32_t items, uint32_t per_block, uint32_t most) { const uint32_t g = (items + per_block - 1) / per_block; return g < 1 ? 1u : g < most ? g : most; }
static int launch_stream_pass(b2_ctx* c, const BatchPtrs& B, cudaStream_t s, uint32_t& launches) {
    const StreamPass& S = c->sp;
    const uint32_t msg_bound = c->small ? c->sm.msgs : c->opt.max_msgs, sms = c->n_sms;
    CU(cudaMemsetAsync(S.cnts, 0, 4 * (16 + 2 * (size_t)S.cap), s));
    CU(cudaEventRecord(c->st_ev[0], s));
    k_stream_route<<<grid(msg_bound, 256, sms * 4), 256, 0, s>>>(B, S); CU(cudaEventRecord(c->st_ev[1], s));
    k_stream_alloc<<<grid(c->st_max, 256, sms), 256, 0, s>>>(B, S); CU(cudaEventRecord(c->st_ev[2], s));
    k_stream_group<<<grid(msg_bound, 256, sms * 4), 256, 0, s>>>(B, S); CU(cudaEventRecord(c->st_ev[3], s));
    k_stream_run<<<grid(c->st_max, 4, sms * 8), 128, 0, s>>>(B, S); CU(cudaEventRecord(c->st_ev[4], s));
    k_stream_rst<<<grid(c->n_runs, 4, sms * 4), 128, 0, s>>>(B, S); CU(cudaEventRecord(c->st_ev[5], s));
    CU(cudaMemcpyAsync(c->h_st_cnts, S.cnts, 64, cudaMemcpyDeviceToHost, s));
    if (c->ring_kind == RingKind::batch_streams) CU(cudaMemsetAsync(S.cnt, 0, 8 * (size_t)S.cap, s));
    launches += 5; c->stream_ran = true; c->st_input = B.bytes;
    return B2_OK;
}

static uint32_t fused_warps(const b2_ctx* c) { return c->avg_frame && !c->dense ? kFusedWarps : kFusedWarpsDense; }
static size_t resolve_smem(const b2_ctx* c, bool fused) { const size_t b = (size_t)c->max_run_tiles * 12; return fused || b > 200 * 1024 ? 0 : b; }

static int launch_pipeline(b2_ctx* c, bool timed = true) {
    const BatchPtrs B = make_ptrs(c);
    DevConfig C = c->cfg;
    const bool fused = c->use_fused && !c->slow_heavy && !c->small && c->input_mode == B2_INPUT_COPY && c->resp_mode == B2_RESP_COPY && c->use_tma_pack &&
                       (((uint64_t)c->nbytes + 255) & ~255ull) + 4096 <= c->opt.max_resp_bytes;
    C.fused = fused ? 1u : 0u; C.ovf_base = (c->nbytes + 255u) & ~255u; c->fused_last = fused;
    cudaStream_t s = c->stream;
    int st = 0; uint32_t launches = 0;
    const bool prof = c->profile_stages;
    auto mark = [&](const char* name) { if (prof) { c->stage_names[st] = name; cudaEventRecord(c->ev[st + 1], s); st++; } };
    const uint32_t mask = c->stage_mask;
    const bool small_launch = c->small && c->use_fused_small && !prof;
    const bool search_zeroes = (mask & 1) && c->n_runs && c->n_tiles && !small_launch;
    if ((mask & 1) && !search_zeroes) CU(cudaMemsetAsync(B.totals, 0, 48, s));
    if (timed) CU(cudaEventRecord(c->ev[0], s));
    c->stream_ran = false;
    if (c->n_runs == 0) { c->n_stages = 0; c->last_launches = 0; return B2_OK; }
    if (small_launch) {
        k_small<<<1, kSmallThreads, sizeof(SmallSmem), s>>>(B, C);
        launches = 1;
        if (c->stream_armed) { int rc = launch_stream_pass(c, B, s, launches); if (rc != B2_OK) return rc; }
        c->stage_names[0] = "fused_small";
        if (timed) cudaEventRecord(c->ev[1], s);
        c->n_stages = timed ? 1 : 0; c->last_launches = launches;
        CU(cudaGetLastError());
        return B2_OK;
    }
    const uint32_t sms = c->n_sms;
    if (mask & 1) {
    if (c->n_tiles) {
        const uint32_t search_threads = fused ? kSearchThreadsFused : 256u;
        k_tile_search<<<(c->n_tiles * 32 + search_threads - 1) / search_threads, search_threads, 0, s>>>(B, C); launches++; mark("tile_search");
        if (C.pull) k_tile_walk_pull<<<(uint32_t)(((uint64_t)c->n_tiles * 8 + 127) / 128), 128, 0, s>>>(B, C);
        else k_tile_walk<<<(c->n_tiles + 127) / 128, 128, 0, s>>>(B, C);
        launches++; mark("tile_walk");
    }
    {
        const size_t smem = resolve_smem(c, fused);
        k_resolve<<<c->n_runs, 256, smem, s>>>(B, C, smem == 0 ? 1u : 0u); launches++; mark("resolve");
    }
    if (fused) {
        const uint32_t fw = fused_warps(c);
        if (c->n_tiles) { k_fused<<<sms, fw * 32, sizeof(FusedWarpSmem) * fw, s>>>(B, C); launches++; mark("fused"); }
    } else {
    if (c->n_tiles) { k_frame_table<<<(uint32_t)(((uint64_t)c->n_tiles * C.spec_k + 255) / 256), 256, 0, s>>>(B, C); launches++; mark("frame_table"); }
    k_decode<<<sms * B2_DECODE_MIN_BLOCKS, kDecodeWarps * 32, 0, s>>>(B, C); launches++; mark("decode");
    k_scan_blocks<<<sms, kScanBlock, 0, s>>>(B); launches++;
    mark("scan");
    }
    }
    if (fused) {
        if (mask & 4) { k_pack_slow<true><<<sms * B2_SLOW_MIN_BLOCKS * (256 / kSlowLiteThreads), kSlowLiteThreads, 0, s>>>(B, C); launches++; mark("pack_slow"); }
    } else if (c->use_tma_pack) {
        if (mask & 4) {
            if (c->slow_heavy || c->cfg.by_ref) { C.verify_done = 1; k_crc_verify<<<sms * 6, 256, 0, s>>>(B, C); launches++; mark("crc_verify"); }
            k_pack_slow<false><<<sms * B2_SLOW_MIN_BLOCKS, 256, 8 * kSnapRing, s>>>(B, C); launches++; mark("pack_slow");
        }
        if (mask & 2) {
            if ((c->avg_frame && c->avg_frame < 640) || c->cfg.by_ref) k_pack_tma<kPackGroupSmall><<<sms, kPackWarps * 32, sizeof(PackWarpSmem) * kPackWarps, s>>>(B, C);
            else k_pack_tma<kPackGroup><<<sms, kPackWarps * 32, sizeof(PackWarpSmem) * kPackWarps, s>>>(B, C);
            launches++; mark("pack");
        }
    } else { k_pack<<<sms * B2_PACK_MIN_BLOCKS, 256, 0, s>>>(B, C); launches++; mark("pack"); }
    if (c->resp_mode == B2_RESP_IOVEC && !c->small) {
        k_emit_iov<<<sms * 4, 256, 0, s>>>(B, c->d_iov, (unsigned long long)(uintptr_t)c->h_resp, (unsigned long long)(uintptr_t)c->host_bytes);
        launches++; mark("emit_iov");
    }
    if (c->stream_armed) { int rc = launch_stream_pass(c, B, s, launches); if (rc != B2_OK) return rc; }
    if (!prof && timed) { c->stage_names[0] = "pipeline"; cudaEventRecord(c->ev[1], s); st = 1; }
    c->n_stages = st; c->last_launches = launches;
    CU(cudaGetLastError());
    return B2_OK;
}

static bool replay_refused(const b2_ctx* c) {
    if (!c || !c->uploaded) { set_err("no batch uploaded"); return true; }
    if (c->stream_armed) { set_err("a submitted batch of a context with a stream table must be collected first: this entry point replays a batch and does not run the stream pass"); return true; }
    return false;
}
extern "C" int b2_batch_execute(b2_ctx* c, float* kernel_ms, uint32_t* n_launches) {
    if (replay_refused(c)) return B2_E_INVAL;
    CU(cudaSetDevice(c->opt.device));
    c->profile_stages = true;
    int rc = launch_pipeline(c);
    c->profile_stages = false;
    if (rc != B2_OK) return rc;
    CU(cudaStreamSynchronize(c->stream));
    float ms = 0.f;
    if (c->n_stages) CU(cudaEventElapsedTime(&ms, c->ev[0], c->ev[c->n_stages]));
    c->last_kernel_ms = ms; c->executed = true;
    if (kernel_ms) *kernel_ms = ms;
    if (n_launches) *n_launches = c->last_launches;
    return B2_OK;
}

extern "C" int b2_batch_execute_many(b2_ctx* c, uint32_t steps, float* total_ms, uint32_t* n_launches) {
    if (steps == 0) { set_err("no batch uploaded"); return B2_E_INVAL; }
    if (replay_refused(c)) return B2_E_INVAL;
    CU(cudaSetDevice(c->opt.device));
    cudaEvent_t e0, e1;
    CU(cudaEventCreate(&e0)); CU(cudaEventCreate(&e1));
    CU(cudaEventRecord(e0, c->stream));
    uint32_t launches = 0;
    for (uint32_t i = 0; i < steps; i++) {
        int rc = launch_pipeline(c);
        if (rc != B2_OK) return rc;
        launches += c->last_launches;
    }
    CU(cudaEventRecord(e1, c->stream));
    CU(cudaStreamSynchronize(c->stream));
    float ms = 0.f;
    CU(cudaEventElapsedTime(&ms, e0, e1));
    cudaEventDestroy(e0); cudaEventDestroy(e1);
    c->executed = true;
    if (c->n_stages) { float t = 0.f; cudaEventElapsedTime(&t, c->ev[0], c->ev[c->n_stages]); c->last_kernel_ms = t; }
    if (total_ms) *total_ms = ms;
    if (n_launches) *n_launches = launches;
    return B2_OK;
}

extern "C" int b2_batch_launch(b2_ctx* c) {
    if (replay_refused(c)) return B2_E_INVAL;
    CU(cudaSetDevice(c->opt.device));
    if (c->first_pending) { CU(cudaEventRecord(c->ev_first, c->stream)); c->first_pending = false; }
    int rc = launch_pipeline(c, false);
    if (rc != B2_OK) return rc;
    CU(cudaEventRecord(c->ev_last, c->stream));
    c->executed = true;
    return B2_OK;
}
extern "C" int b2_batch_wait(b2_ctx* c) {
    if (!c) return B2_E_INVAL;
    CU(cudaSetDevice(c->opt.device));
    CU(cudaStreamSynchronize(c->stream));
    c->first_pending = true;
    return B2_OK;
}
extern "C" int b2_elapsed_ms(b2_ctx* a, b2_ctx* b, float* ms) {
    if (!a || !b || !ms) return B2_E_INVAL;
    CU(cudaSetDevice(a->opt.device));
    CU(cudaEventElapsedTime(ms, a->ev_first, b->ev_last));
    return B2_OK;
}

static void refs_to_iov(b2_ctx* c, b2_batch_result* out, const void* host_bytes) {
    b2_run_status* rs = const_cast<b2_run_status*>(out->runs);
    for (uint32_t r = 0; r < out->n_runs; r++) rs[r].n_unanswered = 0;
    for (uint32_t i = 0; i < out->n_msgs; i++) {
        const b2_msg_desc& d = out->msgs[i];
        b2_iovec a = { const_cast<uint8_t*>(out->resp), 0 }, b = a;
        if (d.status == B2_MSG_ECHOED || d.status == B2_MSG_ERROR_REPLIED) {
            const b2_resp_ref rf = d.status == B2_MSG_ECHOED ? out->refs[i] : b2_resp_ref{0, 0, 0, 0};
            a.iov_base = const_cast<uint8_t*>(out->resp) + d.resp_off; a.iov_len = rf.src_len ? rf.prefix_len : d.resp_len;
            if (rf.src_len) { b.iov_base = const_cast<uint8_t*>(static_cast<const uint8_t*>(host_bytes)) + rf.src_off; b.iov_len = rf.src_len; }
        } else rs[d.run_idx].n_unanswered++;
        c->h_iov[2 * (size_t)i] = a; c->h_iov[2 * (size_t)i + 1] = b;
    }
    out->iov = c->h_iov; out->refs = nullptr;
}

static int download_normal(b2_ctx* c, b2_batch_result* out) {
    CU(cudaMemcpyAsync(c->h_totals, c->d_totals, 48, cudaMemcpyDeviceToHost, c->stream));
    CU(cudaStreamSynchronize(c->stream));
    if (c->n_runs && c->fused_last) {
        const bool heavy = (uint64_t)c->h_totals[3] * 8 > c->h_totals[0];
        if ((c->h_totals[2] & 2u) && !(c->h_totals[2] & 1u)) {
            c->slow_heavy = true;
            int rc = launch_pipeline(c); if (rc != B2_OK) return rc;
            CU(cudaMemcpyAsync(c->h_totals, c->d_totals, 48, cudaMemcpyDeviceToHost, c->stream));
            CU(cudaStreamSynchronize(c->stream));
        }
        c->slow_heavy = heavy || c->slow_heavy;
    } else if (c->n_runs && c->slow_heavy && !c->small) {
        c->slow_heavy = ((uint64_t)c->h_totals[3] + c->h_totals[7]) * 8 > c->h_totals[0];
    }
    if (c->n_runs && (c->h_totals[2] & 3u)) {
        set_err(c->h_totals[2] & 1u ? "more messages than max_msgs" : "responses exceed max_resp_bytes"); return B2_E_CAPACITY;
    }
    if (c->n_runs && c->fused_last) c->h_totals[1] = ((c->nbytes + 255u) & ~255u) + c->h_totals[9];
    const uint32_t n_msgs = c->n_runs ? c->h_totals[0] : 0, resp_bytes = c->n_runs ? c->h_totals[1] : 0;
    if (c->n_runs) CU(cudaMemcpyAsync(c->h_run_status, c->d_run_status, sizeof(b2_run_status) * c->n_runs, cudaMemcpyDeviceToHost, c->stream));
    if (n_msgs) CU(cudaMemcpyAsync(c->h_msgs, c->d_msgs, sizeof(b2_msg_desc) * (size_t)n_msgs, cudaMemcpyDeviceToHost, c->stream));
    if (resp_bytes) CU(cudaMemcpyAsync(c->h_resp, c->d_resp, resp_bytes, cudaMemcpyDeviceToHost, c->stream));
    const bool iovec = c->resp_mode == B2_RESP_IOVEC;
    if (n_msgs && c->cfg.by_ref && !iovec) CU(cudaMemcpyAsync(c->h_refs, c->d_refs, sizeof(b2_resp_ref) * (size_t)n_msgs, cudaMemcpyDeviceToHost, c->stream));
    if (n_msgs && iovec) CU(cudaMemcpyAsync(c->h_iov, c->d_iov, 32 * (size_t)n_msgs, cudaMemcpyDeviceToHost, c->stream));
// ... 438 lines not shown
    else {
        cudaPointerAttributes at; memset(&at, 0, sizeof at);
        if (cudaPointerGetAttributes(&at, bytes) == cudaSuccess && at.type == cudaMemoryTypeHost && at.devicePointer) {
            dev = (unsigned long long)(uintptr_t)at.devicePointer; c->ring_pin_base = bytes; c->ring_pin_dev = dev;
        } else cudaGetLastError();
    }
    if (!dev) { memcpy(slot + c->ring_dev.off_in, bytes, nbytes); dev = (unsigned long long)(uintptr_t)(slot + c->ring_dev.off_in); }
    return dev;
}
static uint8_t* ring_claim(b2_ctx* c, const char* wait_call) {
    if (!c->ring_collected[c->ring_next % kRingSlots]) { set_err("submit ring full: %s the oldest ticket first", wait_call); return nullptr; }
    return ring_slot(c, c->ring_next);
}
static RingSlotHdr* ring_fill(b2_ctx* c, uint8_t* slot, const void* bytes, uint32_t nbytes, const b2_run* runs, uint32_t n_runs) {
    overwrites(c, kDevInput | kDevBatch);
    RingSlotHdr* h = reinterpret_cast<RingSlotHdr*>(slot);
    h->bytes_dev = ring_stage(c, slot, bytes, nbytes);
    if (n_runs) memcpy(slot + c->ring_dev.off_runs, runs, sizeof(b2_run) * (size_t)n_runs);
    h->n_runs = n_runs; h->nbytes = nbytes;
    return h;
}
static int ring_ring(b2_ctx* c, RingSlotHdr* h, const void* bytes, uint32_t* ticket) {
    const uint32_t t = c->ring_next;
    c->ring_bytes[t % kRingSlots] = bytes; c->ring_collected[t % kRingSlots] = false;
    __sync_synchronize();
    h->submit = t;
    __sync_synchronize();
    c->ring_next = t + 1;
    *ticket = t;
    if (!c->ring_ctl[1]) { CU(cudaSetDevice(c->opt.device)); return ring_launch(c); }
    return B2_OK;
}
static int ring_spin(b2_ctx* c, const RingSlotHdr* h, uint32_t ticket) {
    uint64_t spins = 0;
    while (h->done != ticket) {
#if defined(__x86_64__)
        __builtin_ia32_pause();
#endif
        if ((++spins & 0xfffff) == 0) {
            if (!c->ring_ctl[1]) { CU(cudaSetDevice(c->opt.device)); int rc = ring_launch(c); if (rc != B2_OK) return rc; }
            if (cudaStreamQuery(c->ring_stream) != cudaErrorNotReady && h->done != ticket && !c->ring_ctl[1]) continue;
            if (spins > (1ull << 34)) { set_err("ring kernel did not answer"); return B2_E_CUDA; }
        }
    }
    __sync_synchronize();
    return B2_OK;
}
static uint8_t* ring_collect(b2_ctx* c, bool args_ok, uint32_t ticket, const char* bad_ticket, int& rc) {
    rc = B2_E_INVAL;
    if (!args_ok || !c->ring_slots || ticket == 0 || ticket >= c->ring_next || ticket + kRingSlots < c->ring_next) { set_err(bad_ticket); return nullptr; }
    if (c->ring_collected[ticket % kRingSlots]) { set_err("ticket already collected"); return nullptr; }
    const bool in_order = c->ring_kind == RingKind::batch_streams;
    if (in_order && ticket != c->ring_next_wait) { set_err("a context whose ring runs the stream pass collects its tickets in ticket order"); return nullptr; }
    uint8_t* slot = ring_slot(c, ticket);
    if ((rc = ring_spin(c, reinterpret_cast<const RingSlotHdr*>(slot), ticket)) != B2_OK) return nullptr;
    c->ring_collected[ticket % kRingSlots] = true;
    if (in_order) c->ring_next_wait = ticket + 1;
    return slot;
}
extern "C" int b2_ring_stop(b2_ctx* c) { if (!c) return B2_E_INVAL; cudaSetDevice(c->opt.device); ring_halt(c); return B2_OK; }

extern "C" int b2_ring_submit(b2_ctx* c, const void* bytes, uint32_t nbytes, const b2_run* runs, uint32_t n_runs, uint32_t* ticket) {
    if (!c || !bytes || !runs || !ticket || n_runs == 0) { set_err("null argument"); return B2_E_INVAL; }
    if (c->has_streams && c->ring_kind != RingKind::batch_streams) { set_err("the ring path runs the stream pass only after b2_stream_ring_enable: use b2_batch_submit on a context with a stream table"); return B2_E_INVAL; }
    if (c->ring_kind == RingKind::h2_server) { set_err("this context's ring serves h2 (b2_h2_ring_enable): use b2_h2_ring_submit"); return B2_E_INVAL; }
    if (c->ring_kind == RingKind::h2_client) { set_err("this context's ring serves h2 client connections (b2_h2_client_ring_enable): use b2_h2_client_ring_submit"); return B2_E_INVAL; }
    if (nbytes > kSmallBytes || n_runs > kSmallRuns) { set_err("b2_ring_submit serves batches up to 128 KiB / 512 runs: use b2_batch_submit"); return B2_E_CAPACITY; }
    if (!c->ring_slots) { int rc = b2_ring_start(c); if (rc != B2_OK) return rc; }
    uint8_t* slot = ring_claim(c, "b2_ring_wait");
    if (!slot) return B2_E_CAPACITY;
    for (uint32_t r = 0; r < n_runs; r++)
        if ((runs[r].offset & 15u) || (uint64_t)runs[r].offset + runs[r].length > nbytes) { set_err("run offset must be 16-aligned and inside the batch"); return B2_E_INVAL; }
    RingSlotHdr* h = ring_fill(c, slot, bytes, nbytes, runs, n_runs);
    const SmallLayout L = small_layout(nbytes, n_runs, c->opt.max_msgs);
    h->small_msgs = L.msgs; h->small_resp = L.resp; h->off_rs = L.off_rs; h->off_msgs = L.off_msgs;
    h->off_refs = L.off_refs; h->off_resp = L.off_resp; h->total = L.total; h->by_ref = c->cfg.by_ref;
    return ring_ring(c, h, bytes, ticket);
}

extern "C" int b2_ring_wait(b2_ctx* c, uint32_t ticket, b2_batch_result* out) {
    if (c && c->ring_kind == RingKind::h2_server) { set_err("this context's ring serves h2: use b2_h2_ring_wait"); return B2_E_INVAL; }
    if (c && c->ring_kind == RingKind::h2_client) { set_err("this context's ring serves h2 client connections: use b2_h2_client_ring_wait"); return B2_E_INVAL; }
    int rc;
    uint8_t* slot = ring_collect(c, c && out, ticket, "bad ring ticket", rc);
    if (!slot) return rc;
    const uint32_t si = ticket % kRingSlots;
    const bool streams = c->ring_kind == RingKind::batch_streams;
    RingSlotHdr* h = reinterpret_cast<RingSlotHdr*>(slot);
    memset(out, 0, sizeof *out);
    const uint8_t* ob = slot + c->ring_dev.off_out;
    const uint32_t* tot = reinterpret_cast<const uint32_t*>(ob);
    if (tot[2] & 3u) {
        if (!streams && ring_busy(c)) { set_err("ring overflow fallback needs the other tickets collected first"); return B2_E_CAPACITY; }
        if (!streams) ring_halt(c);
        const bool allow = c->allow_small; c->allow_small = false;
        rc = b2_process_batch(c, c->ring_bytes[si], h->nbytes, reinterpret_cast<const b2_run*>(slot + c->ring_dev.off_runs), h->n_runs, out);
        c->allow_small = allow;
        if (streams) { __sync_synchronize(); c->ring_ctl[3] = ticket; __sync_synchronize(); }
        return rc;
    }
    out->runs = reinterpret_cast<const b2_run_status*>(ob + h->off_rs); out->n_runs = h->n_runs;
    out->msgs = reinterpret_cast<const b2_msg_desc*>(ob + h->off_msgs); out->n_msgs = tot[0];
    out->resp = ob + h->off_resp; out->resp_bytes = tot[1];
    out->refs = h->by_ref ? reinterpret_cast<const b2_resp_ref*>(ob + h->off_refs) : nullptr;
    if (c->resp_mode == B2_RESP_IOVEC) refs_to_iov(c, out, c->ring_bytes[si]);
    out->n_launches = 0; out->kernel_ms = 0.f;
    if (streams) { c->stream_valid = true; c->st_view_ticket = ticket; c->st_input = c->d_bytes; }
    note_avg_frame(c, h->nbytes, out->n_msgs);
    return B2_OK;
}
extern "C" uint64_t b2_ring_launches(b2_ctx* c) { return c ? c->ring_launches : 0; }
extern "C" int b2_ring_phase_ns(b2_ctx* c, uint32_t ticket, uint64_t out[4]) {
    if (!c || !c->ring_slots || !out) return B2_E_INVAL;
    const RingSlotHdr* h = reinterpret_cast<const RingSlotHdr*>(ring_slot(c, ticket));
    for (int k = 0; k < 4; k++) out[k] = h->stamps[k + 1] - h->stamps[0];
    return B2_OK;
}

extern "C" int b2_latency_probe(b2_ctx* c, const void* bytes, uint32_t nbytes, const b2_run* runs, uint32_t n_runs, uint32_t iters, int use_ring, float* us_out) {
    if (!c || !us_out) return B2_E_INVAL;
    b2_batch_result res;
    for (uint32_t i = 0; i < iters; i++) {
        timespec t0, t1; clock_gettime(CLOCK_MONOTONIC, &t0);
        int rc;
        if (use_ring) { uint32_t t = 0; rc = b2_ring_submit(c, bytes, nbytes, runs, n_runs, &t); if (rc == B2_OK) rc = b2_ring_wait(c, t, &res); }
        else rc = b2_process_batch(c, bytes, nbytes, runs, n_runs, &res);
        clock_gettime(CLOCK_MONOTONIC, &t1);
        if (rc != B2_OK) return rc;
        if (res.n_msgs == 0) { set_err("latency probe batch produced no messages"); return B2_E_INVAL; }
        us_out[i] = (float)((t1.tv_sec - t0.tv_sec) * 1e6 + (t1.tv_nsec - t0.tv_nsec) * 1e-3);
    }
    return B2_OK;
}

extern "C" int b2_stage_times(b2_ctx* c, const char** names, float* ms, int cap) {
    if (!c) return B2_E_INVAL;
    int n = c->n_stages < cap ? c->n_stages : cap;
    for (int i = 0; i < n; i++) {
        names[i] = c->stage_names[i];
        float t = 0.f;
        cudaEventElapsedTime(&t, c->ev[i], c->ev[i + 1]);
        ms[i] = t;
    }
    int total = c->n_stages;
    if (c->stream_valid && c->stream_ran) {
        for (int i = 0; i < 5; i++, total++) if (total < cap) { names[total] = kStreamStages[i]; float t = 0.f; cudaEventElapsedTime(&t, c->st_ev[i], c->st_ev[i + 1]); ms[total] = t; }
    }
    if (c->sw_ran) {
        for (int i = 0; i < 7; i++, total++) if (total < cap) { names[total] = kSwStages[i]; float t = 0.f; cudaEventElapsedTime(&t, c->sw_ev[i], c->sw_ev[i + 1]); ms[total] = t; }
    }
    return total;
}

extern "C" int b2_batch_info(b2_ctx* c, uint32_t out[4]) {
    if (!c || !out) return B2_E_INVAL;
    out[0] = c->cfg.tile_bytes; out[1] = c->n_tiles; out[2] = c->cfg.spec_k; out[3] = c->fused_last ? 1u : 0u;
    return B2_OK;
}

static uint32_t block_regs(const b2_resident_kernel& k) { return (k.threads + 31) / 32 * ((k.regs * 32 + 255) / 256 * 256); }
static uint32_t smem_step(uint32_t bytes, uint32_t most) {
    static const uint32_t kKB[] = { 0, 8, 16, 32, 64, 100, 132, 164, 196, 228 };
    for (uint32_t kb : kKB) if (kb * 1024 >= bytes) return std::min(kb * 1024, most);
    return most;
}
extern "C" int b2_resident_plan(b2_ctx* c, b2_resident_kernel* out, int cap) {
    if (!c || (!out && cap > 0)) { set_err("null argument"); return B2_E_INVAL; }
    if (!c->plan[kPlanFused].name) { set_err("this build has no function attributes to plan with"); return B2_E_INVAL; }
    b2_resident_kernel k[kPlanKernels];
    memcpy(k, c->plan, sizeof k);
    const uint32_t fw = fused_warps(c);
    k[kPlanFused].threads = fw * 32; k[kPlanFused].smem_bytes += (uint32_t)(sizeof(FusedWarpSmem) * fw);
    k[kPlanResolve].smem_bytes += (uint32_t)resolve_smem(c, true);
    const b2_resident_kernel& f = k[kPlanFused];
    const uint32_t f_regs = block_regs(f), f_smem = f.smem_bytes + c->block_smem_reserve;
    const uint32_t room_regs = c->sm_regs > f_regs ? c->sm_regs - f_regs : 0, f_step = smem_step(f_smem, c->sm_smem);
    const uint32_t room_smem = f_step > f_smem ? f_step - f_smem : 0;
    const uint32_t room_warps = c->sm_warps > fw ? c->sm_warps - fw : 0, room_blocks = c->sm_blocks > 1 ? c->sm_blocks - 1 : 0;
    for (int i = 0; i < kPlanKernels; i++) {
        uint32_t n = room_blocks;
        n = std::min(n, room_regs / std::max(1u, block_regs(k[i])));
        n = std::min(n, room_smem / (k[i].smem_bytes + c->block_smem_reserve));
        n = std::min(n, room_warps / ((k[i].threads + 31) / 32));
        k[i].fits = n;
    }
    for (int i = 0; i < kPlanKernels && i < cap; i++) out[i] = k[i];
    return kPlanKernels;
}

extern "C" int b2_device_pci_bus_id(int device, char* out, int cap) {
    if (!out || cap < 13) return B2_E_INVAL;
    if (cudaDeviceGetPCIBusId(out, cap, device) != cudaSuccess) { cudaGetLastError(); return B2_E_CUDA; }
    return B2_OK;
}

extern "C" int b2_counters_read(b2_ctx* c, int64_t out[B2_N_COUNTERS]) {
    if (!c || !out) return B2_E_INVAL;
    CU(cudaSetDevice(c->opt.device));
    CU(cudaMemcpy(out, c->d_counters, 8 * B2_N_COUNTERS, cudaMemcpyDeviceToHost));
    return B2_OK;
}
extern "C" void* b2_counters_device_ptr(b2_ctx* c) { return c ? (void*)c->d_counters : nullptr; }
extern "C" int b2_counters_allreduce(b2_ctx* c, void* nccl_comm) {
    if (!c || !nccl_comm) { set_err("null argument"); return B2_E_INVAL; }
    typedef int (*allreduce_fn)(const void*, void*, size_t, int, int, void*, cudaStream_t);
    static allreduce_fn fn = reinterpret_cast<allreduce_fn>(dlsym(RTLD_DEFAULT, "ncclAllReduce"));
    if (!fn) { set_err("ncclAllReduce is not loaded in this process"); return B2_E_INVAL; }
    CU(cudaSetDevice(c->opt.device));
    const int rc = fn(c->d_counters, c->d_counters, B2_N_COUNTERS, 4 , 0 , nccl_comm, c->stream);
    if (rc != 0) { char code[16]; snprintf(code, sizeof code, "%d", rc); set_err("ncclAllReduce failed: ncclResult_t %s", code); return B2_E_CUDA; }
    CU(cudaStreamSynchronize(c->stream));
    return B2_OK;
}

extern "C" void* b2_debug_resp_device_ptr(b2_ctx* c) { return c ? (void*)c->d_resp : nullptr; }

__global__ void k_crc32c_batch(const uint8_t* bytes, const uint32_t* offs, const uint32_t* lens, uint32_t n, uint32_t* out,
                               const uint32_t* adv, uint32_t init_crc = 0) {
    __shared__ uint32_t s_hot[kCrcHotWords];
    crc_tabs_to_smem(s_hot, adv);
    CrcTabs ct; ct.hot = s_hot; ct.tree = adv + kCrcHotWords;
    const uint32_t lane = threadIdx.x & 31, n_warps = (gridDim.x * blockDim.x) >> 5;
    for (uint32_t i = (blockIdx.x * blockDim.x + threadIdx.x) >> 5; i < n; i += n_warps) {
        const uint32_t c = warp_crc32c_update(init_crc ^ 0xffffffffu, bytes + offs[i], lens[i], lane, ct) ^ 0xffffffffu;
        if (lane == 0) out[i] = c;
    }
}

static bool out_place(uint64_t& total, uint64_t need, uint32_t out_cap, uint32_t* off) { *off = (uint32_t)total; total += (need + 15) & ~15ull; return total <= out_cap; }
extern "C" int b2_crc32c_batch(b2_ctx* c, const void* bytes, uint32_t nbytes, const uint32_t* offs, const uint32_t* lens,
                               uint32_t n, uint32_t* out) {
    if (!c || !bytes || !offs || !lens || !out) { set_err("null argument"); return B2_E_INVAL; }
    if (h2_ring_refuses(c, false)) return B2_E_INVAL;
    if (nbytes > c->opt.max_batch_bytes || n > c->opt.max_msgs) { set_err("exceeds ctx capacity"); return B2_E_CAPACITY; }
    for (uint32_t i = 0; i < n; i++) if ((uint64_t)offs[i] + lens[i] > nbytes) { set_err("slice outside buffer"); return B2_E_INVAL; }
    CU(cudaSetDevice(c->opt.device));
    overwrites(c, kDevInput | kDevBatch);
    CU(cudaMemcpyAsync(c->d_bytes, bytes, nbytes, cudaMemcpyHostToDevice, c->stream));
    CU(cudaMemcpyAsync(c->d_frame_off, offs, 4 * (size_t)n, cudaMemcpyHostToDevice, c->stream));
    CU(cudaMemcpyAsync(c->d_slot, lens, 4 * (size_t)n, cudaMemcpyHostToDevice, c->stream));
    if (n) k_crc32c_batch<<<c->n_sms * 8, 256, 0, c->stream>>>(c->d_bytes, c->d_frame_off, c->d_slot, n, (uint32_t*)c->d_aux, c->d_crc_adv);
    CU(cudaMemcpyAsync(out, c->d_aux, 4 * (size_t)n, cudaMemcpyDeviceToHost, c->stream));
    CU(cudaStreamSynchronize(c->stream));
    return B2_OK;
}

__global__ void k_snappy_batch(const uint8_t* bytes, const uint32_t* offs, const uint32_t* lens, uint32_t n, uint8_t* out,
                               const uint32_t* out_offs, const uint32_t* out_caps, int32_t* out_lens) {
    const uint32_t lane = threadIdx.x & 31, n_warps = (gridDim.x * blockDim.x) >> 5;
    __shared__ __align__(16) uint8_t s_rings[8 * kSnapRing];
    for (uint32_t i = (blockIdx.x * blockDim.x + threadIdx.x) >> 5; i < n; i += n_warps) {
        uint32_t produced = 0;
        const bool ok = out_caps[i] != 0xffffffffu &&
                        warp_snappy_decode(bytes + offs[i], lens[i], out + out_offs[i], out_caps[i], lane, produced, s_rings + (threadIdx.x >> 5) * kSnapRing);
        if (lane == 0) out_lens[i] = ok ? (int32_t)produced : -1;
    }
}

extern "C" int b2_snappy_uncompress_batch(b2_ctx* c, const void* bytes, uint32_t nbytes, const uint32_t* offs, const uint32_t* lens,
                                          uint32_t n, void* out, uint32_t out_cap, uint32_t* out_offs, int32_t* out_lens) {
    if (!c || !bytes || !offs || !lens || !out || !out_offs || !out_lens) { set_err("null argument"); return B2_E_INVAL; }
    if (h2_ring_refuses(c, false)) return B2_E_INVAL;
    if (nbytes > c->opt.max_batch_bytes || n > c->opt.max_msgs || out_cap > c->opt.max_resp_bytes) { set_err("exceeds ctx capacity"); return B2_E_CAPACITY; }
    std::vector<uint32_t> caps(n);
    uint64_t total = 0;
    for (uint32_t i = 0; i < n; i++) {
        if ((uint64_t)offs[i] + lens[i] > nbytes) { set_err("slice outside buffer"); return B2_E_INVAL; }
        const uint8_t* p = (const uint8_t*)bytes + offs[i];
        uint32_t v = 0, shift = 0, k = 0; bool ok = false;
        while (k < lens[i] && shift < 32) { const uint32_t b = p[k++]; v |= (b & 0x7f) << shift; if (b < 128) { ok = true; break; } shift += 7; }
        const bool valid = ok && (uint64_t)v <= 32ull * lens[i] + 64ull;
        caps[i] = valid ? v : 0xffffffffu;
        if (!out_place(total, valid ? v : 0, out_cap, &out_offs[i])) { set_err("output exceeds out_cap"); return B2_E_CAPACITY; }
    }
    CU(cudaSetDevice(c->opt.device));
    uint32_t* d_offs = c->d_frame_off; uint32_t* d_lens = c->d_slot; uint32_t* d_ooffs = c->d_frame_run;
    uint32_t* d_caps = (uint32_t*)c->d_jobs; int32_t* d_olens = (int32_t*)c->d_aux;
    overwrites(c, kDevInput | kDevBatch);
    CU(cudaMemcpyAsync(c->d_bytes, bytes, nbytes, cudaMemcpyHostToDevice, c->stream));
    CU(cudaMemcpyAsync(d_offs, offs, 4 * (size_t)n, cudaMemcpyHostToDevice, c->stream));
    CU(cudaMemcpyAsync(d_lens, lens, 4 * (size_t)n, cudaMemcpyHostToDevice, c->stream));
    CU(cudaMemcpyAsync(d_ooffs, out_offs, 4 * (size_t)n, cudaMemcpyHostToDevice, c->stream));
    CU(cudaMemcpyAsync(d_caps, caps.data(), 4 * (size_t)n, cudaMemcpyHostToDevice, c->stream));
    if (n) k_snappy_batch<<<c->n_sms * 4, 256, 0, c->stream>>>(c->d_bytes, d_offs, d_lens, n, c->d_unz, d_ooffs, d_caps, d_olens);
    CU(cudaMemcpyAsync(out_lens, d_olens, 4 * (size_t)n, cudaMemcpyDeviceToHost, c->stream));
    if (total) CU(cudaMemcpyAsync(out, c->d_unz, total, cudaMemcpyDeviceToHost, c->stream));
    CU(cudaStreamSynchronize(c->stream));
    return B2_OK;
}

__global__ void __launch_bounds__(256) k_snappy_compress_batch(const uint8_t* bytes, const uint32_t* offs, const uint32_t* lens, uint32_t n,
                                                               uint8_t* out, const uint32_t* out_offs, uint32_t* out_lens, uint16_t* tabs) {
    const uint32_t lane = threadIdx.x & 31, n_warps = (gridDim.x * blockDim.x) >> 5, warp = (blockIdx.x * blockDim.x + threadIdx.x) >> 5;
    uint16_t* table = tabs + (size_t)(warp % kSnappyWarps) * kSnappyMaxTable;
    for (uint32_t i = warp; i < n; i += n_warps) {
        const uint32_t c = warp_snappy_compress(bytes + offs[i], lens[i], out + out_offs[i], table, lane);
        if (lane == 0) out_lens[i] = c;
    }
}

extern "C" int b2_snappy_compress_batch(b2_ctx* c, const void* bytes, uint32_t nbytes, const uint32_t* offs, const uint32_t* lens,
                                        uint32_t n, void* out, uint32_t out_cap, uint32_t* out_offs, uint32_t* out_lens) {
    if (!c || !bytes || !offs || !lens || !out || !out_offs || !out_lens) { set_err("null argument"); return B2_E_INVAL; }
    if (h2_ring_refuses(c, false)) return B2_E_INVAL;
    if (nbytes > c->opt.max_batch_bytes || n > c->opt.max_msgs || out_cap > c->opt.max_resp_bytes) { set_err("exceeds ctx capacity"); return B2_E_CAPACITY; }
    uint64_t total = 0;
    for (uint32_t i = 0; i < n; i++) {
        if ((uint64_t)offs[i] + lens[i] > nbytes) { set_err("slice outside buffer"); return B2_E_INVAL; }
        if (!out_place(total, snappy_max_compressed_length(lens[i]), out_cap, &out_offs[i])) { set_err("output exceeds out_cap"); return B2_E_CAPACITY; }
    }
    CU(cudaSetDevice(c->opt.device));
    uint32_t* d_offs = c->d_frame_off; uint32_t* d_lens = c->d_slot; uint32_t* d_ooffs = c->d_frame_run; uint32_t* d_olens = (uint32_t*)c->d_aux;
    overwrites(c, kDevInput | kDevBatch);
    CU(cudaMemcpyAsync(c->d_bytes, bytes, nbytes, cudaMemcpyHostToDevice, c->stream));
    CU(cudaMemcpyAsync(d_offs, offs, 4 * (size_t)n, cudaMemcpyHostToDevice, c->stream));
    CU(cudaMemcpyAsync(d_lens, lens, 4 * (size_t)n, cudaMemcpyHostToDevice, c->stream));
    CU(cudaMemcpyAsync(d_ooffs, out_offs, 4 * (size_t)n, cudaMemcpyHostToDevice, c->stream));
    if (n) k_snappy_compress_batch<<<c->n_sms * 4, 256, 0, c->stream>>>(c->d_bytes, d_offs, d_lens, n, c->d_unz, d_ooffs, d_olens, c->d_snappy_tab);
    CU(cudaMemcpyAsync(out_lens, d_olens, 4 * (size_t)n, cudaMemcpyDeviceToHost, c->stream));
    if (total) CU(cudaMemcpyAsync(out, c->d_unz, total, cudaMemcpyDeviceToHost, c->stream));
    CU(cudaStreamSynchronize(c->stream));
    return B2_OK;
}


static std::mutex g_leaf_mu;
// ... 665 lines not shown
```

### brpc_b200/csrc/b2_kernels.cuh

```cuda
#pragma once
#include <cuda_runtime.h>
#include "b2_core.cuh"
#include "b2_inflate.cuh"

namespace b2 {

enum TileKind : uint8_t { kRanOff = 0, kStop = 1, kAmbig = 2 };

struct __align__(16) TileRec {
    uint32_t entry;
    uint32_t exit;
    uint32_t count;
    uint8_t kind;
    int8_t last_proto;
    uint8_t live;
    int8_t pf_in;
};

struct __align__(16) MsgAux {
    uint32_t msg_off;
    uint32_t msg_len;
    uint32_t att_len;
    uint32_t att_off;
    uint32_t cks_off;
    uint32_t cks_len;
    uint32_t svc_off, svc_len;
    uint32_t mth_off, mth_len;
    uint32_t pad;
    uint32_t err_kind;
};
struct __align__(16) PackJob {
    uint32_t src_off;
    uint32_t bulk_len;
    uint16_t head_len;
    uint8_t pad;
    uint8_t fast;
    uint32_t slot_len;
};
constexpr uint32_t kHeadBytes = 96;

enum ErrKind : uint32_t { kErrNone = 0, kErrAttachment, kErrNoService, kErrNoMethod, kErrParseRequest };

struct DevMethod {
    char full_method[200];
    uint32_t full_method_len;
    char service_short[64];  uint32_t service_short_len;
    char service_full[120];  uint32_t service_full_len;
    char request_type[96];   uint32_t request_type_len;
    int32_t handler, echo_attachment, response_checksum_type, response_compress_type;
};
struct DevConfig {
    uint64_t max_body_size;
    uint32_t tile_bytes, tile_shift;
    uint32_t n_methods;
    uint32_t identity_len;
    uint32_t stream_handler;
    uint32_t spec_k;
    uint32_t by_ref;
    uint32_t verify_done;
    uint32_t proto_mask;
    uint32_t fused;
    uint32_t ovf_base;
    uint32_t pull_vecs;
    uint32_t pull;
    char identity[64];
};

struct BatchPtrs {
    const uint8_t* bytes;
    const b2_run* runs;
    const uint32_t* run_tile_base;
    const uint4* tile_info;
    TileRec* tiles;
    uint32_t* tile_base;
    uint32_t* tile_scratch;
    uint32_t* tile_spec;
    b2_run_status* run_status;
    uint32_t* frame_off;
    uint32_t* frame_run;
    uint32_t* frame_row;
    uint4* rows;
    b2_msg_desc* msgs;
    MsgAux* aux;
    PackJob* jobs;
    uint4* refs;
    uint32_t* slow_idx;
    uint8_t* heads;
    uint32_t* slot;
    uint32_t* scan_tmp;
    uint8_t* resp;
    uint8_t* unz;
    uint16_t* snappy_tab;
    unsigned long long* counters;
    uint32_t* totals;
    const DevMethod* methods;
    const uint32_t* crc_adv;
    uint32_t n_runs, n_tiles, max_msgs, max_resp;
};

template <bool kSpec, typename Emit>
B2_HD void walk_tile(const uint8_t* run, uint32_t len, uint32_t entry, int pf_in, uint32_t tile_end,
                     uint64_t max_body, bool client, TileRec& t, Emit emit, uint32_t mask = kProtoMaskDefault) {
    uint32_t pos = entry, count = 0;
    int pf = kSpec ? -1 : pf_in, last = 0;
    uint8_t kind = kRanOff;
    while (pos < tile_end) {
        const Step s = cut_input_message(run, len, pos, pf, max_body, client, mask);
        if (kSpec && count == 0 && (s.popped || (s.index != 12 && nshead_claims(run, len, pos, max_body, mask)))) { kind = kAmbig; break; }
        if (s.err != B2_PARSE_OK) { kind = kStop; break; }
        emit(count, s);
        count++; last = s.index; pf = s.index; pos = s.new_pos;
    }
    t.entry = entry; t.exit = pos; t.count = count; t.kind = kind; t.last_proto = (int8_t)last;
}
struct NoEmit { B2_HD void operator()(uint32_t, const Step&) const {} };
constexpr uint32_t kSpecK = 16;
constexpr uint32_t kSpecKDense = 128;
constexpr uint8_t kKindRewalked = 0x80;
struct EmitSpec {
    uint32_t* out; uint32_t run_off, cap;
    __device__ __forceinline__ void operator()(uint32_t i, const Step& s) const {
        if (i < cap) out[i] = (run_off + s.frame_pos) | ((uint32_t)(s.index != 1) << 31);
    }
};

#if defined(__CUDACC__)

__device__ __forceinline__ uint32_t find_run(const uint32_t* base, uint32_t n_runs, uint32_t tile) {
    uint32_t lo = 0, hi = n_runs;
    while (hi - lo > 1) { const uint32_t mid = (lo + hi) >> 1; if (__ldg(base + mid) <= tile) lo = mid; else hi = mid; }
    return lo;
}
__device__ __forceinline__ bool is_magic(uint32_t w) { return w == kMagicPRPC || w == kMagicSTRM; }
#ifndef B2_SEARCH_FIRST
#define B2_SEARCH_FIRST 2
#endif

constexpr uint32_t kSearchThreadsFused = 128;
__global__ void __launch_bounds__(256, 6) k_tile_search(BatchPtrs B, DevConfig C) {
    const uint32_t warp = (blockIdx.x * blockDim.x + threadIdx.x) >> 5, lane = threadIdx.x & 31;
    if (blockIdx.x == 0 && threadIdx.x < 12) B.totals[threadIdx.x] = 0;
    if (warp >= B.n_tiles) return;
    const uint4 ti = __ldg(B.tile_info + warp);
    const uint32_t k = ti.z;
    const uint8_t* base = B.bytes + ti.x;
    const uint32_t len = ti.y;
    uint32_t entry = kNone;
    if (k == 0) {
        entry = 0;
    } else {
        const uint32_t t0 = k << C.tile_shift;
        const uint32_t t1 = min(t0 + C.tile_bytes, len);
        for (uint32_t c0 = t0; c0 < t1 && entry == kNone; c0 += (c0 == t0 ? 512u * B2_SEARCH_FIRST : 2048u)) {
            const int nwin = c0 == t0 ? B2_SEARCH_FIRST : 4;
            uint4 v[4]; uint32_t nx[4];
            #pragma unroll
            for (int u = 0; u < 4; u++) {
                const uint32_t p0 = c0 + u * 512 + lane * 16;
                v[u] = make_uint4(0, 0, 0, 0); nx[u] = 0;
                if (u < nwin && p0 < t1) {
                    v[u] = __ldg(reinterpret_cast<const uint4*>(base + p0));
                    nx[u] = __ldg(reinterpret_cast<const uint32_t*>(base + p0 + 16));
                }
            }
            #pragma unroll
            for (int u = 0; u < 4; u++) {
                if (entry != kNone || u >= nwin) break;
                const uint32_t w0 = c0 + u * 512, p0 = w0 + lane * 16;
                const uint32_t w[5] = { v[u].x, v[u].y, v[u].z, v[u].w, nx[u] };
                uint32_t mask = 0, mkind = 0;
                const bool ext = (C.proto_mask & ((1u << 3) | (1u << 4))) != 0;
                #pragma unroll
                for (int k4 = 0; k4 < 4; k4++) {
                    uint32_t e = __vcmpeq4(w[k4], 0x50505050u) | __vcmpeq4(w[k4], 0x53535353u);
                    if (ext) e |= __vcmpeq4(w[k4], 0x48484848u);
                    while (e) {
                        const int b = (__ffs(e) - 1) >> 3;
                        e &= ~(0xffu << (8 * b));
                        const int j = 4 * k4 + b;
                        const uint32_t word = __funnelshift_r(w[k4], w[k4 + 1], b * 8);
                        const bool other = ext && ((word == kMagicHULU && (C.proto_mask & 8u)) || (word == kMagicSOFA && (C.proto_mask & 16u)));
                        if ((is_magic(word) || other) && p0 + j + 4 <= len && p0 + j < t1) { mask |= 1u << j; if (other) mkind |= (word == kMagicHULU ? 1u : 2u) << (2 * j); }
                    }
                }
                uint32_t any = __ballot_sync(0xffffffffu, mask != 0);
                const uint32_t n5 = __shfl_down_sync(0xffffffffu, v[u].y, 1), n6 = __shfl_down_sync(0xffffffffu, v[u].z, 1);
                while (any && entry == kNone) {
                    const int src = __ffs(any) - 1;
                    uint32_t m = __shfl_sync(0xffffffffu, mask, src);
                    const uint32_t kinds = __shfl_sync(0xffffffffu, mkind, src);
                    while (m && entry == kNone) {
                        const int jj = __ffs(m) - 1;
                        const uint32_t p = w0 + src * 16 + jj;
                        m &= m - 1;
                        const uint32_t kind = (kinds >> (2 * jj)) & 3u;
                        if (kind == 2) { entry = p; break; }
                        uint32_t body_le = 0, meta_le = 0;
                        if (src < 31) {
                            const uint32_t q = (uint32_t)(jj + 4) >> 2, sh = ((uint32_t)(jj + 4) & 3u) * 8u;
                            const uint32_t a1 = w[1], a2 = w[2], a3 = w[3], a4 = w[4];
                            const uint32_t x0 = q == 1 ? a1 : q == 2 ? a2 : q == 3 ? a3 : a4;
                            const uint32_t x1 = q == 1 ? a2 : q == 2 ? a3 : q == 3 ? a4 : n5;
                            const uint32_t x2 = q == 1 ? a3 : q == 2 ? a4 : q == 3 ? n5 : n6;
                            body_le = __shfl_sync(0xffffffffu, __funnelshift_r(x0, x1, sh), src);
                            meta_le = __shfl_sync(0xffffffffu, __funnelshift_r(x1, x2, sh), src);
                        } else if (p + 12 <= len) {
                            body_le = load_le32(base + p + 4); meta_le = load_le32(base + p + 8);
                        } else continue;
                        const uint32_t body = kind == 1 ? body_le : __byte_perm(body_le, 0, 0x0123), meta = kind == 1 ? meta_le : __byte_perm(meta_le, 0, 0x0123);
                        if (meta <= body && (uint64_t)body <= C.max_body_size) entry = p;
                    }
                    any &= any - 1;
                }
            }
        }
    }
    if (lane == 0) B.tiles[warp].entry = entry;
}

struct HdrWords { uint32_t w0, w1, w2, w3; };
__device__ __forceinline__ HdrWords load_hdr_words(const uint8_t* p) {
    const uint32_t* q = reinterpret_cast<const uint32_t*>((uintptr_t)p & ~(uintptr_t)3);
    HdrWords h; h.w0 = __ldg(q); h.w1 = __ldg(q + 1); h.w2 = __ldg(q + 2); h.w3 = __ldg(q + 3);
    return h;
}
template <typename Emit>
__device__ __forceinline__ void walk_tile_spec(const uint8_t* run, uint32_t len, uint32_t entry, uint32_t tile_end,
                                               uint64_t max_body, bool client, TileRec& t, Emit emit, uint32_t mask) {
    uint32_t pos = entry, count = 0, prev_len = 0, pre_pos = kNone;
    int pf = -1, last = 0;
    uint8_t kind = kRanOff;
    HdrWords pre; pre.w0 = pre.w1 = pre.w2 = pre.w3 = 0;
    while (pos < tile_end) {
        Step s;
        bool fast = false;
        if (len - pos >= 12) {
            const HdrWords h = pre_pos == pos ? pre : load_hdr_words(run + pos);
            const uint32_t guess = pos + prev_len;
            if (prev_len && guess < tile_end && (uint64_t)guess + 12 <= len) { pre = load_hdr_words(run + guess); pre_pos = guess; }
            else pre_pos = kNone;
            const uint32_t sh = 8u * (pos & 3u);
            const uint32_t h0 = sh ? __funnelshift_r(h.w0, h.w1, sh) : h.w0, h1 = sh ? __funnelshift_r(h.w1, h.w2, sh) : h.w1,
                           h2 = sh ? __funnelshift_r(h.w2, h.w3, sh) : h.w2;
            const int idx = h0 == kMagicPRPC ? 1 : h0 == kMagicSTRM ? 2 : 0;
            const uint32_t body = __byte_perm(h1, 0, 0x0123), meta = __byte_perm(h2, 0, 0x0123);
            if (idx && ((mask >> idx) & 1u) && pf != 12 && (uint64_t)body <= max_body && (uint64_t)(len - pos) >= 12ull + body && meta <= body) {
                s.err = B2_PARSE_OK; s.index = idx; s.pf = idx; s.frame_pos = pos; s.new_pos = pos + 12 + body; s.body = body; s.meta = meta; s.popped = false;
                fast = true;
            }
        }
        if (!fast) s = cut_input_message(run, len, pos, pf, max_body, client, mask);
        if (count == 0 && (s.popped || (s.index != 12 && nshead_claims(run, len, pos, max_body, mask)))) { kind = kAmbig; break; }
        if (s.err != B2_PARSE_OK) { kind = kStop; break; }
        emit(count, s);
        count++; last = s.index; pf = s.index; prev_len = s.new_pos - pos; pos = s.new_pos;
    }
    t.entry = entry; t.exit = pos; t.count = count; t.kind = kind; t.last_proto = (int8_t)last;
}

__global__ void __launch_bounds__(128) k_tile_walk(BatchPtrs B, DevConfig C) {
    const uint32_t t = blockIdx.x * blockDim.x + threadIdx.x;
    if (t >= B.n_tiles) return;
    const uint4 ti = __ldg(B.tile_info + t);
    const uint32_t k = ti.z;
    b2_run run; run.offset = ti.x; run.length = ti.y; run.flags = ti.w >> 24;
    TileRec rec;
    rec.entry = B.tiles[t].entry; rec.exit = 0; rec.count = 0; rec.kind = kStop; rec.last_proto = 0; rec.live = 0; rec.pf_in = -1;
    if (rec.entry != kNone) {
        EmitSpec e; e.out = B.tile_spec + (size_t)t * C.spec_k; e.run_off = run.offset; e.cap = C.spec_k;
        walk_tile_spec(B.bytes + run.offset, run.length, rec.entry, (k + 1) << C.tile_shift, C.max_body_size, (run.flags & B2_RUN_CLIENT) != 0, rec, e, run_mask(C.proto_mask, run.flags));
    }
    B.tiles[t] = rec;
}

__global__ void __launch_bounds__(128) k_tile_walk_pull(BatchPtrs B, DevConfig C) {
    const uint32_t g = blockIdx.x * blockDim.x + threadIdx.x;
    const uint32_t t = g >> 3, sub = threadIdx.x & 7u, lane = threadIdx.x & 31u;
    if (t >= B.n_tiles) return;
    const uint32_t gmask = 0xffu << (lane & 24u), l0 = lane & 24u;
    const uint4 ti = __ldg(B.tile_info + t);
    const uint32_t k = ti.z, len = ti.y;
    const uint8_t* run = B.bytes + ti.x;
    const bool client = ((ti.w >> 24) & B2_RUN_CLIENT) != 0;
    const uint32_t pmask = run_mask(C.proto_mask, ti.w >> 24);
    const uint32_t tile_end = (k + 1) << C.tile_shift, cap = C.spec_k;
    uint32_t* spec = B.tile_spec + (size_t)t * cap;
    uint4* rows = B.rows + (size_t)t * cap * 8;
    TileRec rec;
    rec.entry = B.tiles[t].entry; rec.exit = 0; rec.count = 0; rec.kind = kStop; rec.last_proto = 0; rec.live = 0; rec.pf_in = -1;
    if (rec.entry != kNone) {
        uint32_t pos = rec.entry, count = 0; int pf = -1, last = 0; uint8_t kind = kRanOff;
        while (pos < tile_end) {
            bool fast = false; uint32_t new_pos = pos, frame_pos = pos; int idx = 0, err = B2_PARSE_OK; bool popped = false;
            uint4 v = make_uint4(0, 0, 0, 0);
            if (len - pos >= 12) {
                if (sub < C.pull_vecs) v = __ldg(reinterpret_cast<const uint4*>(run + (pos & ~15u)) + sub);
                const uint32_t a0 = __shfl_sync(gmask, v.x, l0), a1 = __shfl_sync(gmask, v.y, l0), a2 = __shfl_sync(gmask, v.z, l0), a3 = __shfl_sync(gmask, v.w, l0);
                const uint32_t b0 = __shfl_sync(gmask, v.x, l0 + 1), b1 = __shfl_sync(gmask, v.y, l0 + 1), b2 = __shfl_sync(gmask, v.z, l0 + 1);
                const uint32_t q = (pos & 15u) >> 2, sh = 8u * (pos & 3u);
                const uint32_t w0 = q == 0 ? a0 : q == 1 ? a1 : q == 2 ? a2 : a3, w1 = q == 0 ? a1 : q == 1 ? a2 : q == 2 ? a3 : b0;
                const uint32_t w2 = q == 0 ? a2 : q == 1 ? a3 : q == 2 ? b0 : b1, w3 = q == 0 ? a3 : q == 1 ? b0 : q == 2 ? b1 : b2;
                const uint32_t h0 = sh ? __funnelshift_r(w0, w1, sh) : w0, h1 = sh ? __funnelshift_r(w1, w2, sh) : w1, h2 = sh ? __funnelshift_r(w2, w3, sh) : w2;
                idx = h0 == kMagicPRPC ? 1 : h0 == kMagicSTRM ? 2 : 0;
                const uint32_t body = __byte_perm(h1, 0, 0x0123), meta = __byte_perm(h2, 0, 0x0123);
                if (idx && ((pmask >> idx) & 1u) && pf != 12 && (uint64_t)body <= C.max_body_size && (uint64_t)(len - pos) >= 12ull + body && meta <= body) { fast = true; new_pos = pos + 12 + body; }
            }
            if (count == 0 && ((pmask >> 12) & 1u)) {
                int amb = 0;
                if (sub == 0) amb = nshead_claims(run, len, pos, C.max_body_size, pmask) ? 1 : 0;
                if (__shfl_sync(gmask, amb, l0)) { kind = kAmbig; break; }
            }
            if (!fast) {
                Step s; s.err = 0; s.index = 0; s.new_pos = 0; s.frame_pos = 0; s.popped = false;
                if (sub == 0) s = cut_input_message(run, len, pos, pf, C.max_body_size, client, pmask);
                err = __shfl_sync(gmask, s.err, l0); idx = __shfl_sync(gmask, s.index, l0); new_pos = __shfl_sync(gmask, s.new_pos, l0);
                frame_pos = __shfl_sync(gmask, s.frame_pos, l0); popped = __shfl_sync(gmask, (int)s.popped, l0) != 0;
                if (count == 0 && popped) { kind = kAmbig; break; }
                if (err != B2_PARSE_OK) { kind = kStop; break; }
                if (sub < C.pull_vecs) v = __ldg(reinterpret_cast<const uint4*>(run + (frame_pos & ~15u)) + sub);
            }
            if (count < cap) {
                if (sub == 0) spec[count] = (ti.x + frame_pos) | ((uint32_t)(idx != 1) << 31);
                if (sub < C.pull_vecs) rows[(size_t)count * 8 + sub] = v;
            }
            count++; last = idx; pf = idx; pos = new_pos;
        }
        rec.exit = pos; rec.count = count; rec.kind = kind; rec.last_proto = (int8_t)last;
    }
    if (sub == 0) B.tiles[t] = rec;
}

__device__ __forceinline__ void run_prefix_body(const BatchPtrs& B, uint32_t* s_warp, uint32_t* s_carry) {
    const uint32_t lane = threadIdx.x & 31, wid = threadIdx.x >> 5, nw = blockDim.x >> 5;
    if (threadIdx.x == 0) *s_carry = 0;
    __syncthreads();
    for (uint32_t base = 0; base < B.n_runs; base += blockDim.x) {
        const uint32_t i = base + threadIdx.x;
        uint32_t v = i < B.n_runs ? __ldcg(&B.run_status[i].n_msgs) : 0, x = v;
        #pragma unroll
        for (int d = 1; d < 32; d <<= 1) { const uint32_t y = __shfl_up_sync(0xffffffffu, x, d); if (lane >= (uint32_t)d) x += y; }
        if (lane == 31) s_warp[wid] = x;
        __syncthreads();
        uint32_t wbase = 0, wtot = 0;
        for (uint32_t w = 0; w < nw; w++) { const uint32_t t = s_warp[w]; if (w < wid) wbase += t; wtot += t; }
        const uint32_t carry = *s_carry;
        if (i < B.n_runs) B.run_status[i].first_msg = carry + wbase + x - v;
        __syncthreads();
        if (threadIdx.x == 0) *s_carry = carry + wtot;
        __syncthreads();
    }
    if (threadIdx.x == 0) { B.totals[0] = *s_carry; if (*s_carry > B.max_msgs) B.totals[2] |= 1u; }
}

constexpr uint32_t kLinkOk = 0x80000000u;
constexpr uint32_t kLinkStop = 0x40000000u;
constexpr uint32_t kLinkEnd = 0x20000000u;
constexpr uint32_t kLinkBroken = 0x10000000u;
constexpr uint32_t kLinkRewalk = 0x08000000u;

__device__ __forceinline__ uint32_t make_link(const TileRec& t, const TileRec* tiles, uint32_t nt, uint32_t shift) {
    if (t.entry == kNone || t.kind == kAmbig) return kLinkRewalk;
    if (t.kind == kStop) return kLinkStop;
    const uint32_t j = t.exit >> shift;
    if (j >= nt) return kLinkEnd;
    return (tiles[j].entry == t.exit ? kLinkOk : kLinkBroken) | j;
}

__global__ void __launch_bounds__(256) k_resolve(BatchPtrs B, DevConfig C, uint32_t use_scratch) {
    extern __shared__ uint32_t sm[];
    const uint32_t r = blockIdx.x;
    const b2_run run = B.runs[r];
    const uint8_t* base = B.bytes + run.offset;
    const uint32_t len = run.length;
    const uint32_t tb = B.run_tile_base[r], nt = B.run_tile_base[r + 1] - tb;
    TileRec* tiles = B.tiles + tb;
    const bool fits = !use_scratch;
    uint32_t* link = fits ? sm : B.tile_scratch + 3ull * tb;
    uint32_t* cp = link + nt;
    uint32_t* live = cp + nt;
    __shared__ uint32_t s_final_pos, s_warp_sum[8], s_warp_pf[8], s_carry_sum, s_carry_pf;
    const uint32_t rmask = run_mask(C.proto_mask, run.flags);
    const bool pf_decides = (run.flags & B2_RUN_CLIENT) && !(rmask & kProtoMaskDump) && (rmask & ~((1u << B2_PROTOCOL_BAIDU_STD) | (1u << B2_PROTOCOL_STREAMING_RPC))) != 0;
    for (uint32_t k = threadIdx.x; k < nt; k += blockDim.x) {
        const TileRec t = tiles[k];
        link[k] = ((k == 0 && t.entry != 0) || pf_decides) ? kLinkRewalk : make_link(t, tiles, nt, C.tile_shift);
        cp[k] = (t.count << 4) | ((uint32_t)t.last_proto & 15u);
        live[k] = 0;
    }
    __shared__ uint32_t s_first_bad;
    if (threadIdx.x == 0) s_first_bad = nt ? nt - 1 : 0;
    __syncthreads();
    {
        uint32_t mine = nt;
        for (uint32_t k = threadIdx.x; k + 1 < nt; k += blockDim.x)
            if (link[k] != (kLinkOk | (k + 1))) { mine = k; break; }
        if (mine < nt) atomicMin(&s_first_bad, mine);
    }
    __syncthreads();
    const uint32_t first_bad = s_first_bad;
    for (uint32_t k = threadIdx.x; k < first_bad; k += blockDim.x) live[k] = 1;
    __syncthreads();
    if (threadIdx.x == 0) {
        uint32_t k = first_bad, pos = 0;
        bool via_ok = first_bad > 0;
        while (k < nt) {
            uint32_t v = link[k];
            if (v & kLinkRewalk) {
                if (via_ok) pos = tiles[k].entry;
                int pf = run.preferred_proto;
                for (uint32_t j = k; j-- > 0;) if (live[j] && (cp[j] >> 4)) { pf = (int)(cp[j] & 15u); break; }
                TileRec t; t.live = 0; t.pf_in = 0;
                walk_tile<false>(base, len, pos, pf, (k + 1) << C.tile_shift, C.max_body_size, (run.flags & B2_RUN_CLIENT) != 0, t, NoEmit(), run_mask(C.proto_mask, run.flags));
                tiles[k].entry = t.entry; tiles[k].exit = t.exit; tiles[k].count = t.count; tiles[k].kind = t.kind | kKindRewalked; tiles[k].last_proto = t.last_proto;
                cp[k] = (t.count << 4) | ((uint32_t)t.last_proto & 15u);
// ... 2643 lines not shown
```

### include/b2rpc.h

```cpp
#ifndef B2RPC_H_
#define B2RPC_H_

#include <stddef.h>
#include <stdint.h>

#ifdef __cplusplus
extern "C" {
#endif

#define B2_OK              0
#define B2_E_INVAL        -1
#define B2_E_NO_DEVICE    -2
#define B2_E_CUDA         -3
#define B2_E_CAPACITY     -4
#define B2_E_NOMEM        -5

#define B2_PARSE_OK                    0
#define B2_PARSE_ERROR_TRY_OTHERS      1
#define B2_PARSE_ERROR_NOT_ENOUGH_DATA 2
#define B2_PARSE_ERROR_TOO_BIG_DATA    3
#define B2_PARSE_ERROR_NO_RESOURCE     4
#define B2_PARSE_ERROR_ABSOLUTELY_WRONG 5

#define B2_PROTOCOL_UNKNOWN       0
// ... 35 lines not shown
#define B2_HAS_CORRELATION_ID   (1u << 3)
#define B2_HAS_ATTACHMENT_SIZE  (1u << 4)
#define B2_HAS_CHUNK_INFO       (1u << 5)
#define B2_HAS_AUTH_DATA        (1u << 6)
#define B2_HAS_STREAM_SETTINGS  (1u << 7)
#define B2_HAS_USER_FIELDS      (1u << 8)
#define B2_HAS_CONTENT_TYPE     (1u << 9)
#define B2_HAS_CHECKSUM_TYPE    (1u << 10)
#define B2_HAS_CHECKSUM_VALUE   (1u << 11)
#define B2_HAS_LOG_ID           (1u << 12)
#define B2_HAS_TRACE_ID         (1u << 13)
#define B2_HAS_REQUEST_ID       (1u << 14)
#define B2_HAS_TIMEOUT_MS       (1u << 15)
#define B2_SHAS_STREAM_ID        (1u << 0)
#define B2_SHAS_SOURCE_STREAM_ID (1u << 1)
#define B2_SHAS_FRAME_TYPE       (1u << 2)
#define B2_SHAS_HAS_CONTINUATION (1u << 3)
#define B2_SHAS_FEEDBACK         (1u << 4)
#define B2_SVAL_HAS_CONTINUATION (1u << 8)

typedef struct b2_run {
    uint64_t socket_id;
    uint32_t offset;
    uint32_t length;
    int32_t  preferred_proto;
    uint32_t flags;
} b2_run;
#define B2_RUN_RPC_DUMP 4u
#define B2_RUN_CLIENT 1u

typedef struct b2_run_status {
    uint32_t consumed;
    uint32_t parse_error;
    uint32_t n_msgs;
    uint32_t first_msg;
    int32_t  preferred_proto;
    uint32_t n_unanswered;
    uint32_t resp_off;
    uint32_t resp_bytes;
} b2_run_status;

typedef struct b2_msg_desc {
    uint32_t run_idx;
    uint32_t frame_off;
    uint32_t body_size;
    uint32_t meta_size;
    int64_t  correlation_id;
    int64_t  log_id;
    int32_t  attachment_size;
    int32_t  compress_type;
    int32_t  checksum_type;
    int32_t  error_code;
    uint16_t has_bits;
    uint8_t  protocol;
    uint8_t  content_type;
    int16_t  method_idx;
    uint16_t status;
    uint32_t resp_off;
    uint32_t resp_len;
} b2_msg_desc;

#define B2_HANDLER_HOST 0
#define B2_HANDLER_ECHO 1

typedef struct b2_method {
    const char* service_full_name;
    const char* service_name;
    const char* method_name;
    const char* request_type_name;
    int32_t handler;
    int32_t echo_attachment;
    int32_t response_checksum_type;
    int32_t response_compress_type;
} b2_method;

typedef struct b2_options {
    int32_t  device;
    uint32_t max_batch_bytes;
    uint32_t max_msgs;
    uint32_t max_runs;
    uint32_t max_resp_bytes;
    uint32_t tile_bytes;
    uint64_t max_body_size;
} b2_options;

typedef struct b2_resp_ref { uint32_t prefix_len, src_off, src_len, reserved; } b2_resp_ref;

typedef struct b2_iovec { void* iov_base; size_t iov_len; } b2_iovec;

typedef struct b2_batch_result {
    const b2_run_status* runs;     uint32_t n_runs;
    const b2_msg_desc*   msgs;     uint32_t n_msgs;
    const uint8_t*       resp;     uint32_t resp_bytes;
    float kernel_ms;
    uint32_t n_launches;
    const b2_resp_ref*   refs;
    const b2_iovec*      iov;
} b2_batch_result;

typedef struct b2_ctx b2_ctx;

int  b2_ctx_create(const b2_options* opt, b2_ctx** out);
void b2_ctx_destroy(b2_ctx* ctx);
const char* b2_last_error(void);
const char* b2_version(void);

int  b2_register_method(b2_ctx* ctx, const b2_method* m);

int  b2_set_protocols(b2_ctx* ctx, uint32_t protocol_mask);

#define B2_STREAM_DESC_ONLY         0
#define B2_STREAM_SNAPPY_UNCOMPRESS 1
int  b2_set_stream_handler(b2_ctx* ctx, int kind);

int  b2_set_server_identity(b2_ctx* ctx, const char* ip_port);

void* b2_block_alloc(size_t size);
void  b2_block_free(void* p);
uint64_t b2_block_pool_host_allocs(void);

#define B2_INPUT_COPY 0
#define B2_INPUT_PULL 1
#define B2_RESP_COPY   0
#define B2_RESP_BY_REF 1
#define B2_RESP_IOVEC  2
int  b2_set_modes(b2_ctx* ctx, int input_mode, int resp_mode);

int  b2_process_batch(b2_ctx* ctx, const void* bytes, uint32_t nbytes,
                      const b2_run* runs, uint32_t n_runs, b2_batch_result* out);

int  b2_batch_submit(b2_ctx* ctx, const void* bytes, uint32_t nbytes, const b2_run* runs, uint32_t n_runs);
int  b2_batch_collect(b2_ctx* ctx, b2_batch_result* out);

int  b2_ring_start(b2_ctx* ctx);
int  b2_ring_stop(b2_ctx* ctx);
int  b2_ring_submit(b2_ctx* ctx, const void* bytes, uint32_t nbytes, const b2_run* runs, uint32_t n_runs, uint32_t* ticket);
int  b2_ring_wait(b2_ctx* ctx, uint32_t ticket, b2_batch_result* out);
uint64_t b2_ring_launches(b2_ctx* ctx);
int  b2_ring_phase_ns(b2_ctx* ctx, uint32_t ticket, uint64_t out[4]);
int  b2_latency_probe(b2_ctx* ctx, const void* bytes, uint32_t nbytes, const b2_run* runs, uint32_t n_runs,
                      uint32_t iters, int use_ring, float* us_out);

int  b2_batch_upload(b2_ctx* ctx, const void* bytes, uint32_t nbytes,
                     const b2_run* runs, uint32_t n_runs);
int  b2_batch_execute(b2_ctx* ctx, float* kernel_ms, uint32_t* n_launches);
int  b2_batch_download(b2_ctx* ctx, b2_batch_result* out);
int  b2_batch_execute_many(b2_ctx* ctx, uint32_t steps, float* total_ms, uint32_t* n_launches);

int  b2_batch_launch(b2_ctx* ctx);
int  b2_batch_wait(b2_ctx* ctx);
int  b2_elapsed_ms(b2_ctx* a, b2_ctx* b, float* ms);

int  b2_batch_info(b2_ctx* ctx, uint32_t out[4]);

typedef struct b2_resident_kernel {
    const char* name;
    uint32_t regs, threads, smem_bytes, fits;
} b2_resident_kernel;
int  b2_resident_plan(b2_ctx* ctx, b2_resident_kernel* out, int cap);

int  b2_device_pci_bus_id(int device, char* out, int cap);

int  b2_stage_times(b2_ctx* ctx, const char** names, float* ms, int cap);

int  b2_crc32c_batch(b2_ctx* ctx, const void* bytes, uint32_t nbytes,
                     const uint32_t* offs, const uint32_t* lens, uint32_t n,
                     uint32_t* out);

int  b2_snappy_uncompress_batch(b2_ctx* ctx, const void* bytes, uint32_t nbytes,
                                const uint32_t* offs, const uint32_t* lens, uint32_t n,
                                void* out, uint32_t out_cap, uint32_t* out_offs, int32_t* out_lens);

int  b2_snappy_compress_batch(b2_ctx* ctx, const void* bytes, uint32_t nbytes,
                              const uint32_t* offs, const uint32_t* lens, uint32_t n,
                              void* out, uint32_t out_cap, uint32_t* out_offs, uint32_t* out_lens);

uint32_t b2_crc32c_extend(uint32_t init_crc, const char* data, size_t n);
size_t   b2_snappy_max_compressed_length(size_t source_bytes);
void     b2_snappy_raw_compress(const char* input, size_t input_length, char* compressed, size_t* compressed_length);
int      b2_snappy_get_uncompressed_length(const char* compressed, size_t compressed_length, size_t* result);
int      b2_snappy_raw_uncompress(const char* compressed, size_t compressed_length, char* uncompressed);

#define B2_REQ_BAIDU_STD     0
#define B2_REQ_STREAM_FRAME  1
#define B2_REQ_HAS_LOG_ID            1u
#define B2_REQ_HAS_TIMEOUT           2u
#define B2_REQ_HAS_SOURCE_STREAM_ID  1u
#define B2_REQ_HAS_CONTINUATION      2u
#define B2_REQ_CONTINUATION_VALUE    4u
typedef struct b2_request {
    uint32_t kind, flags;
    int32_t  method_idx;
    int32_t  timeout_ms;
    int64_t  correlation_id;
    int64_t  log_id;
    int32_t  compress_type, checksum_type;
    int32_t  frame_type;
    uint32_t payload_off, payload_len;
    uint32_t attachment_off, attachment_len;
    uint32_t reserved;
} b2_request;
int  b2_pack_requests(b2_ctx* ctx, const void* bytes, uint32_t nbytes, const b2_request* reqs, uint32_t n,
                      void* out, uint32_t out_cap, uint32_t* out_offs, uint32_t* out_lens);

#define B2_RSP_HAS_STREAM         1u
#define B2_RSP_STREAM_NEED_FEEDBACK 2u
#define B2_RSP_STREAM_WRITABLE    4u
typedef struct b2_reply {
    uint32_t flags;
    int32_t  error_code;
    int64_t  correlation_id;
    int32_t  compress_type, checksum_type, content_type;
    uint32_t error_text_off, error_text_len;
    uint32_t body_off, body_len;
    uint32_t attachment_off, attachment_len;
    uint32_t checksum_value_off, checksum_value_len;
    uint32_t extra_streams_off, n_extra_streams;
    uint32_t user_fields_off, n_user_fields;
    uint32_t reserved;
    int64_t  stream_id;
} b2_reply;
int  b2_pack_responses(b2_ctx* ctx, const void* bytes, uint32_t nbytes, const b2_reply* replies, uint32_t n,
                       void* out, uint32_t out_cap, uint32_t* out_offs, uint32_t* out_lens);

#define B2_RUN_H2_PREFACE 2u
typedef struct b2_h2_frame { uint8_t type, flags; uint16_t pad; uint32_t stream_id, payload_off, payload_len; } b2_h2_frame;
int  b2_h2_scan_batch(b2_ctx* ctx, const void* bytes, uint32_t nbytes, const b2_run* runs, uint32_t n_runs,
                      uint32_t max_frame_size, b2_h2_frame* frames, uint32_t cap_per_run,
                      uint32_t* n_frames, uint32_t* consumed, uint32_t* err);
#define B2_HPACK_MAX_CONNS 4096
typedef struct b2_hpack_block { uint32_t conn, offset, length, reserved; } b2_hpack_block;
int  b2_hpack_reset(b2_ctx* ctx, uint32_t conn, uint32_t max_table_size);
int  b2_hpack_decode_batch(b2_ctx* ctx, const void* bytes, uint32_t nbytes, const b2_hpack_block* blocks, uint32_t n_blocks,
                           void* out, uint32_t per_block_cap, uint32_t* out_lens, int32_t* status, uint32_t* n_headers);

#define B2_H2_MAX_CONNS 1024
#define B2_H2_MAX_PENDING 8
#define B2_H2_STREAM_BYTES 69632
int  b2_h2_configure(b2_ctx* ctx, uint32_t max_conns, uint32_t max_pending, uint32_t stream_bytes);
#define B2_H2_HEADER_BYTES 4096
#define B2_H2_FLAG_GRPC            1u
#define B2_H2_FLAG_GRPC_PREFIX_OK  2u
#define B2_H2_FLAG_GRPC_COMPRESSED 4u
#define B2_H2_FLAG_HAS_PATH        8u
#define B2_H2_FLAG_BODY_IN_INPUT  16u
#define B2_H2_NO_METHOD 255u
typedef struct b2_h2_run_status {
    uint32_t consumed, parse_error, n_msgs, first_msg;
    uint32_t ctrl_off, ctrl_len;
    uint32_t remote_max_frame_size, remote_stream_window_size;
} b2_h2_run_status;
typedef struct b2_h2_msg {
    uint32_t run_idx, stream_id;
    uint32_t headers_off, headers_len, n_headers;
    uint32_t body_off, body_len;
    uint32_t http_method;
    uint32_t content_type;
    uint32_t flags;
    int32_t  method_idx;
    uint32_t msg_off, msg_len;
    uint32_t path_off, path_len;
    uint32_t reserved;
} b2_h2_msg;
int  b2_h2_conn_reset(b2_ctx* ctx, uint32_t conn);
int  b2_h2_process_batch(b2_ctx* ctx, const void* bytes, uint32_t nbytes, const b2_run* runs, uint32_t n_runs,
                         b2_h2_run_status* rs, b2_h2_msg* msgs, uint32_t msg_cap, uint32_t* n_msgs,
                         void* out, uint32_t out_cap);

#define B2_H2_RESP_GRPC 1u
#define B2_H2_RESP_BODY_IN_INPUT 2u
#define B2_H2_RESP_BODY_IN_OUT   4u
#define B2_H2_RESP_CT_IN_OUT     8u
typedef struct b2_h2_response {
    uint32_t conn, stream_id;
    int32_t  status_code;
    uint32_t flags;
    uint32_t content_type_off, content_type_len;
    uint32_t body_off, body_len;
    int32_t  grpc_status;
    uint32_t grpc_message_off, grpc_message_len;
    uint32_t reserved;
} b2_h2_response;
int  b2_h2_pack_responses(b2_ctx* ctx, const void* bytes, uint32_t nbytes, const b2_h2_response* resps, uint32_t n,
                          void* out, uint32_t out_cap, uint32_t* out_offs, uint32_t* out_lens);

#define B2_H2_REQ_GRPC       1u
#define B2_H2_REQ_GET        2u
#define B2_H2_REQ_HTTPS      4u
#define B2_H2_REQ_ACCEPT     8u
#define B2_H2_REQ_USER_AGENT 16u
#define B2_H2_REQ_OK     0
#define B2_H2_REQ_ELIMIT 1
#define B2_H2_REQ_RUNOUT 2
#define B2_H2_REQ_LOGOFF 3
#define B2_H2_REQ_NO_ROOM 4
typedef struct b2_h2_request {
    uint32_t conn, flags;
    uint32_t path_off, path_len;
    uint32_t authority_off, authority_len;
    uint32_t content_type_off, content_type_len;
    uint32_t body_off, body_len;
    uint32_t extra_off, extra_len;
} b2_h2_request;
typedef struct b2_h2_request_result { int32_t status; uint32_t stream_id, out_off, out_len; } b2_h2_request_result;
int  b2_h2_pack_requests(b2_ctx* ctx, const void* bytes, uint32_t nbytes, const b2_h2_request* reqs, uint32_t n,
                         void* out, uint32_t out_cap, b2_h2_request_result* results);
// ... 157 lines not shown
```

Measured before the change: 1.075 billion.

## Group consecutive tiles per walk thread, searching only group head tiles

Adds a walk-group mode in which one thread walks several consecutive tiles of a run, continuing from the previous tile's exit position. Only the first tile of each group goes through tile_search. This cuts search work and launch width, and lets the header prefetch carry across tile boundaries. Auto mode enables groups of 2 on the fused, non-dense path. The cost is less parallelism in the walk, a longer serial chain per thread, extra metadata upload, and changed launch bounds on k_tile_walk.

```diff
diff --git a/brpc_b200/abi.py b/brpc_b200/abi.py
--- a/brpc_b200/abi.py
+++ b/brpc_b200/abi.py
@@ -142,6 +142,8 @@
     l.b2_set_server_identity.argtypes = [C.c_void_p, C.c_char_p]
     l.b2_set_stream_handler.argtypes = [C.c_void_p, C.c_int]
     l.b2_set_protocols.argtypes = [C.c_void_p, C.c_uint32]
+    l.b2_set_walk_group.argtypes = [C.c_void_p, C.c_uint32]
+    l.b2_walk_group.argtypes = [C.c_void_p]
     l.b2_block_alloc.restype = C.c_void_p; l.b2_block_alloc.argtypes = [C.c_size_t]
     l.b2_block_free.argtypes = [C.c_void_p]
     l.b2_block_pool_host_allocs.restype = C.c_uint64
@@ -223,7 +225,7 @@
 ABI_SYMBOLS = ["b2_ctx_create", "b2_ctx_destroy", "b2_last_error", "b2_version", "b2_register_method",
                "b2_set_server_identity", "b2_set_stream_handler", "b2_set_protocols", "b2_block_alloc", "b2_block_free", "b2_block_pool_host_allocs", "b2_set_modes", "b2_ring_start", "b2_ring_stop", "b2_ring_submit", "b2_ring_wait", "b2_ring_launches", "b2_ring_phase_ns", "b2_latency_probe", "b2_process_batch", "b2_batch_submit", "b2_batch_collect", "b2_batch_upload",
                "b2_batch_execute", "b2_batch_execute_many", "b2_batch_download", "b2_batch_launch", "b2_batch_wait",
-               "b2_elapsed_ms", "b2_batch_info", "b2_resident_plan", "b2_device_pci_bus_id", "b2_stage_times", "b2_crc32c_batch", "b2_crc32c_extend", "b2_snappy_max_compressed_length", "b2_snappy_raw_compress", "b2_snappy_get_uncompressed_length", "b2_snappy_raw_uncompress", "b2_snappy_uncompress_batch", "b2_snappy_compress_batch", "b2_hpack_reset", "b2_hpack_decode_batch", "b2_pack_requests", "b2_pack_responses", "b2_h2_scan_batch", "b2_h2_conn_reset", "b2_h2_configure", "b2_h2_process_batch", "b2_h2_pack_responses", "b2_counters_read",
+               "b2_elapsed_ms", "b2_batch_info", "b2_set_walk_group", "b2_walk_group", "b2_resident_plan", "b2_device_pci_bus_id", "b2_stage_times", "b2_crc32c_batch", "b2_crc32c_extend", "b2_snappy_max_compressed_length", "b2_snappy_raw_compress", "b2_snappy_get_uncompressed_length", "b2_snappy_raw_uncompress", "b2_snappy_uncompress_batch", "b2_snappy_compress_batch", "b2_hpack_reset", "b2_hpack_decode_batch", "b2_pack_requests", "b2_pack_responses", "b2_h2_scan_batch", "b2_h2_conn_reset", "b2_h2_configure", "b2_h2_process_batch", "b2_h2_pack_responses", "b2_counters_read",
                "b2_counters_device_ptr", "b2_counters_allreduce", "b2_h2_pack_requests", "b2_h2_conn_set_next_stream_id", "b2_h2_conn_peer_update",
                "b2_h2_client_conn_reset", "b2_h2_client_process_batch", "b2_h2_client_abandon_streams", "b2_h2_conn_set_gunzip",
                "b2_h2_serve_batch", "b2_stream_configure", "b2_stream_open", "b2_stream_set_connected", "b2_stream_close", "b2_stream_query",
@@ -386,6 +388,12 @@
 
     def set_protocols(self, mask):
         _check(lib.b2_set_protocols(self._h, mask))
+
+    def set_walk_group(self, mode):
+        _check(lib.b2_set_walk_group(self._h, mode))
+
+    def walk_group(self):
+        return _check(lib.b2_walk_group(self._h))
 
     def set_modes(self, input_mode=INPUT_COPY, resp_mode=RESP_COPY):
         _check(lib.b2_set_modes(self._h, input_mode, resp_mode))
diff --git a/brpc_b200/csrc/b2_api.cu b/brpc_b200/csrc/b2_api.cu
--- a/brpc_b200/csrc/b2_api.cu
+++ b/brpc_b200/csrc/b2_api.cu
@@ -50,7 +50,7 @@
     DevConfig cfg;
     std::vector<DevMethod> methods;
     uint8_t* d_bytes = nullptr; b2_run* d_runs = nullptr; uint32_t* d_run_tile_base = nullptr;
-    TileRec* d_tiles = nullptr; uint32_t* d_tile_base = nullptr; uint32_t* d_tile_scratch = nullptr; uint32_t* d_tile_spec = nullptr; b2_run_status* d_run_status = nullptr;
+    TileRec* d_tiles = nullptr; uint32_t* d_tile_base = nullptr; uint32_t* d_tile_scratch = nullptr; TileRec* d_head_recs = nullptr; uint32_t* d_tile_spec = nullptr; b2_run_status* d_run_status = nullptr;
     uint32_t* d_frame_off = nullptr; uint32_t* d_frame_run = nullptr; b2_msg_desc* d_msgs = nullptr; MsgAux* d_aux = nullptr; PackJob* d_jobs = nullptr; uint32_t* d_slow_idx = nullptr; uint8_t* d_heads = nullptr;
     uint32_t* d_slot = nullptr; uint32_t* d_scan_tmp = nullptr; uint8_t* d_resp = nullptr; uint8_t* d_unz = nullptr; uint16_t* d_snappy_tab = nullptr; HpackState* d_hpack = nullptr; H2Conn* d_h2 = nullptr; H2Stream* d_h2_streams = nullptr; uint8_t* d_h2_slots = nullptr; uint32_t h2_max_conns = B2_H2_MAX_CONNS, h2_pending = B2_H2_MAX_PENDING, h2_stream_bytes = B2_H2_STREAM_BYTES; uint64_t h2_last_in = 0, h2_last_out = 0;
     uint32_t* d_frame_row = nullptr; uint4* d_rows = nullptr;
@@ -86,6 +86,7 @@
     cudaEvent_t ev_first = nullptr, ev_last = nullptr; bool first_pending = true;
     bool profile_stages = false; bool allow_small = true; bool use_fused = true; bool fused_last = false; bool slow_heavy = false;
     bool adaptive_tile = false; bool dense = false; uint32_t avg_frame = 0;
+    uint32_t walk_group_mode = 0, walk_group = 1, n_groups = 0, walk_group_last = 1; size_t meta_group_off = 0;
     uint8_t* d_meta = nullptr; uint8_t* h_meta = nullptr;
     uint8_t* d_small = nullptr; uint8_t* h_small = nullptr;
     bool small = false, small_copy_queued = false, use_fused_small = true; SmallLayout sm = {};
@@ -172,7 +173,7 @@
     if (c->ring_slots) cudaFreeHost(c->ring_slots);
     if (c->ring_ctl) cudaFreeHost((void*)c->ring_ctl);
     cudaFree(c->d_ring_ticket);
-    cudaFree(c->d_bytes); cudaFree(c->d_runs); cudaFree(c->d_run_tile_base); cudaFree(c->d_tiles); cudaFree(c->d_tile_base); cudaFree(c->d_tile_scratch); cudaFree(c->d_tile_spec);
+    cudaFree(c->d_bytes); cudaFree(c->d_runs); cudaFree(c->d_run_tile_base); cudaFree(c->d_tiles); cudaFree(c->d_tile_base); cudaFree(c->d_tile_scratch); cudaFree(c->d_head_recs); cudaFree(c->d_tile_spec);
     cudaFree(c->d_run_status); cudaFree(c->d_frame_off); cudaFree(c->d_frame_run); cudaFree(c->d_msgs); cudaFree(c->d_aux); cudaFree(c->d_jobs); cudaFree(c->d_slow_idx); cudaFree(c->d_heads); cudaFree(c->d_slot);
     cudaFree(c->d_scan_tmp); cudaFree(c->d_resp); cudaFree(c->d_unz); cudaFree(c->d_snappy_tab); cudaFree(c->d_refs); cudaFree(c->d_iov); cudaFreeHost(c->h_iov); cudaFree(c->d_frame_row); cudaFree(c->d_rows); cudaFreeHost(c->h_refs); cudaFree(c->d_hpack); cudaFree(c->d_h2); cudaFree(c->d_h2_streams); cudaFree(c->d_h2_slots); cudaFree(c->d_h2_gz_merge); cudaFree(c->d_counters); cudaFree(c->d_totals); cudaFree(c->d_methods); cudaFree(c->d_crc_adv); cudaFree(c->d_meta); cudaFree(c->d_small); cudaFreeHost(c->h_meta); cudaFreeHost(c->h_small);
     cudaFreeHost(c->h_run_status); cudaFreeHost(c->h_msgs); cudaFreeHost(c->h_resp); cudaFreeHost(c->h_totals);
@@ -221,6 +222,7 @@
     ALLOC(c->d_tiles, sizeof(TileRec) * (size_t)c->max_tiles);
     ALLOC(c->d_tile_base, 4 * (size_t)c->max_tiles);
     ALLOC(c->d_tile_scratch, 12 * (size_t)c->max_tiles);
+    ALLOC(c->d_head_recs, sizeof(TileRec) * (size_t)c->max_tiles);
     {
         size_t dense_tiles = (size_t)o->max_batch_bytes / 2048 + o->max_runs + 1; if (dense_tiles > c->max_tiles) dense_tiles = c->max_tiles;
         size_t words = (size_t)kSpecK * c->max_tiles; if ((size_t)kSpecKDense * dense_tiles > words) words = (size_t)kSpecKDense * dense_tiles;
@@ -246,9 +248,9 @@
     ALLOC(c->d_totals, 64);
     ALLOC(c->d_methods, sizeof(DevMethod) * 64);
     ALLOC(c->d_crc_adv, (kCrcHotWords + kCrcTreeWords) * 4);
-    ALLOC(c->d_meta, (size_t)o->max_runs * 28 + 16 * (size_t)c->max_tiles + 64);
+    ALLOC(c->d_meta, (size_t)o->max_runs * 28 + 36 * (size_t)c->max_tiles + 64);
     ALLOC(c->d_small, kSmallBlock);
-    HALLOC(c->h_meta, (size_t)o->max_runs * 28 + 16 * (size_t)c->max_tiles + 64);
+    HALLOC(c->h_meta, (size_t)o->max_runs * 28 + 36 * (size_t)c->max_tiles + 64);
     HALLOC(c->h_small, kSmallBlock);
     HALLOC(c->h_run_status, sizeof(b2_run_status) * (size_t)o->max_runs);
     HALLOC(c->h_msgs, sizeof(b2_msg_desc) * (size_t)o->max_msgs);
@@ -387,6 +389,8 @@
     B.runs = reinterpret_cast<const b2_run*>(c->d_meta);
     B.run_tile_base = reinterpret_cast<const uint32_t*>(c->d_meta + (size_t)c->n_runs * sizeof(b2_run));
     B.tile_info = reinterpret_cast<const uint4*>(c->d_meta + c->meta_tile_off);
+    B.group_heads = reinterpret_cast<const uint32_t*>(c->d_meta + c->meta_group_off + 16 * (size_t)c->n_groups); B.head_recs = c->d_head_recs;
+    B.n_groups = c->n_groups; B.walk_group = 1;
     if (c->input_mode == B2_INPUT_PULL) B.bytes = c->pull_bytes;
     if (c->small) {
         B.refs = reinterpret_cast<uint4*>(c->d_small + c->sm.off_refs);
@@ -397,6 +401,16 @@
         B.max_msgs = c->sm.msgs; B.max_resp = c->sm.resp;
     }
     return B;
+}
+
+static bool takes_fused(const b2_ctx* c) {
+    return c->use_fused && !c->slow_heavy && !c->small && c->input_mode == B2_INPUT_COPY && c->resp_mode == B2_RESP_COPY && c->use_tma_pack &&
+           (((uint64_t)c->nbytes + 255) & ~255ull) + 4096 <= c->opt.max_resp_bytes;
+}
+static uint32_t pick_walk_group(const b2_ctx* c) {
+    if (c->input_mode == B2_INPUT_PULL || c->walk_group_mode == 1) return 1;
+    if (c->walk_group_mode >= 2) return c->walk_group_mode;
+    return takes_fused(c) && c->avg_frame && !c->dense ? 2u : 1u;
 }
 
 extern "C" int b2_batch_upload(b2_ctx* c, const void* bytes, uint32_t nbytes, const b2_run* runs, uint32_t n_runs) {
@@ -434,9 +448,15 @@
     c->h_run_tile_base[n_runs] = (uint32_t)nt;
     if (nt > c->max_tiles) { set_err("too many tiles"); return B2_E_CAPACITY; }
     c->n_runs = n_runs; c->n_tiles = (uint32_t)nt; c->nbytes = nbytes; c->max_run_tiles = max_rt; c->host_bytes = bytes;
+    c->small = c->allow_small && nbytes <= kSmallBytes && n_runs <= kSmallRuns && n_runs > 0;
+    c->walk_group = pick_walk_group(c);
     const size_t tile_off = ((size_t)n_runs * sizeof(b2_run) + 4 * ((size_t)n_runs + 1) + 15) & ~(size_t)15;
-    const size_t meta_bytes = tile_off + 16 * (size_t)nt;
-    c->meta_tile_off = tile_off;
+    c->meta_tile_off = tile_off; c->meta_group_off = tile_off + 16 * (size_t)nt;
+    uint32_t ng = 0;
+    if (c->walk_group > 1)
+        for (uint32_t r = 0; r < n_runs; r++) ng += (c->h_run_tile_base[r + 1] - c->h_run_tile_base[r] + c->walk_group - 1) / c->walk_group;
+    c->n_groups = ng;
+    const size_t meta_bytes = c->meta_group_off + 20 * (size_t)ng;
     if (n_runs) memcpy(c->h_meta, runs, (size_t)n_runs * sizeof(b2_run));
     memcpy(c->h_meta + (size_t)n_runs * sizeof(b2_run), c->h_run_tile_base, 4 * ((size_t)n_runs + 1));
     {
@@ -445,6 +465,12 @@
             const uint32_t t0 = c->h_run_tile_base[r], t1 = c->h_run_tile_base[r + 1];
             for (uint32_t t = t0; t < t1; t++) { uint32_t* q = ti + 4 * (size_t)t; q[0] = runs[r].offset; q[1] = runs[r].length; q[2] = t - t0; q[3] = r | (runs[r].flags << 24); }
         }
+        uint32_t* hi = reinterpret_cast<uint32_t*>(c->h_meta + c->meta_group_off);
+        uint32_t* heads = hi + 4 * (size_t)ng;
+        uint32_t g = 0;
+        if (c->walk_group > 1)
+            for (uint32_t r = 0; r < n_runs; r++)
+                for (uint32_t t = c->h_run_tile_base[r]; t < c->h_run_tile_base[r + 1]; t += c->walk_group, g++) { memcpy(hi + 4 * (size_t)g, ti + 4 * (size_t)t, 16); heads[g] = t; }
     }
     overwrites(c, kDevInput | kDevBatch);
     if (c->input_mode == B2_INPUT_PULL) {
@@ -455,7 +481,6 @@
         c->pull_bytes = static_cast<const uint8_t*>(dp);
     } else if (nbytes) CU(cudaMemcpyAsync(c->d_bytes, bytes, nbytes, cudaMemcpyHostToDevice, c->stream));
     CU(cudaMemcpyAsync(c->d_meta, c->h_meta, meta_bytes, cudaMemcpyHostToDevice, c->stream));
-    c->small = c->allow_small && nbytes <= kSmallBytes && n_runs <= kSmallRuns && n_runs > 0;
     if (c->small) c->sm = small_layout(nbytes, n_runs, c->opt.max_msgs);
     if (const char* e = getenv("B2_STAGE_MASK")) c->stage_mask = (uint32_t)atoi(e);
     c->uploaded = true;
@@ -484,10 +509,11 @@
 static size_t resolve_smem(const b2_ctx* c, bool fused) { const size_t b = (size_t)c->max_run_tiles * 12; return fused || b > 200 * 1024 ? 0 : b; }
 
 static int launch_pipeline(b2_ctx* c, bool timed = true) {
-    const BatchPtrs B = make_ptrs(c);
+    BatchPtrs B = make_ptrs(c);
     DevConfig C = c->cfg;
-    const bool fused = c->use_fused && !c->slow_heavy && !c->small && c->input_mode == B2_INPUT_COPY && c->resp_mode == B2_RESP_COPY && c->use_tma_pack &&
-                       (((uint64_t)c->nbytes + 255) & ~255ull) + 4096 <= c->opt.max_resp_bytes;
+    const bool fused = takes_fused(c);
+    B.walk_group = fused || c->walk_group_mode >= 2 ? c->walk_group : 1u;
+    c->walk_group_last = B.walk_group;
     C.fused = fused ? 1u : 0u; C.ovf_base = (c->nbytes + 255u) & ~255u; c->fused_last = fused;
     cudaStream_t s = c->stream;
     int st = 0; uint32_t launches = 0;
@@ -514,8 +540,11 @@
     if (mask & 1) {
     if (c->n_tiles) {
         const uint32_t search_threads = fused ? kSearchThreadsFused : 256u;
-        k_tile_search<<<(c->n_tiles * 32 + search_threads - 1) / search_threads, search_threads, 0, s>>>(B, C); launches++; mark("tile_search");
+        BatchPtrs S = B;
+        if (B.walk_group > 1) { S.tile_info = reinterpret_cast<const uint4*>(c->d_meta + c->meta_group_off); S.tiles = B.head_recs; S.n_tiles = c->n_groups; }
+        k_tile_search<<<(S.n_tiles * 32 + search_threads - 1) / search_threads, search_threads, 0, s>>>(S, C); launches++; mark("tile_search");
         if (C.pull) k_tile_walk_pull<<<(uint32_t)(((uint64_t)c->n_tiles * 8 + 127) / 128), 128, 0, s>>>(B, C);
+        else if (B.walk_group > 1) k_tile_walk<<<(c->n_groups + kWalkGroupThreads - 1) / kWalkGroupThreads, kWalkGroupThreads, 0, s>>>(B, C);
         else k_tile_walk<<<(c->n_tiles + 127) / 128, 128, 0, s>>>(B, C);
         launches++; mark("tile_walk");
     }
@@ -1260,6 +1289,15 @@
     return total;
 }
 
+extern "C" int b2_set_walk_group(b2_ctx* c, uint32_t mode) {
+    if (!c || mode > 8) { set_err("walk group mode: 0 auto, 1 off, 2..8 tiles per group"); return B2_E_INVAL; }
+    c->walk_group_mode = mode;
+    overwrites(c, kDevBatch);
+    return B2_OK;
+}
+
+extern "C" int b2_walk_group(b2_ctx* c) { return c ? (int)c->walk_group_last : B2_E_INVAL; }
+
 extern "C" int b2_batch_info(b2_ctx* c, uint32_t out[4]) {
     if (!c || !out) return B2_E_INVAL;
     out[0] = c->cfg.tile_bytes; out[1] = c->n_tiles; out[2] = c->cfg.spec_k; out[3] = c->fused_last ? 1u : 0u;
@@ -1280,6 +1318,7 @@
     const uint32_t fw = fused_warps(c);
     k[kPlanFused].threads = fw * 32; k[kPlanFused].smem_bytes += (uint32_t)(sizeof(FusedWarpSmem) * fw);
     k[kPlanResolve].smem_bytes += (uint32_t)resolve_smem(c, true);
+    if (c->walk_group > 1) k[kPlanWalk].threads = kWalkGroupThreads;
     const b2_resident_kernel& f = k[kPlanFused];
     const uint32_t f_regs = block_regs(f), f_smem = f.smem_bytes + c->block_smem_reserve;
     const uint32_t room_regs = c->sm_regs > f_regs ? c->sm_regs - f_regs : 0, f_step = smem_step(f_smem, c->sm_smem);
diff --git a/brpc_b200/csrc/b2_kernels.cuh b/brpc_b200/csrc/b2_kernels.cuh
--- a/brpc_b200/csrc/b2_kernels.cuh
+++ b/brpc_b200/csrc/b2_kernels.cuh
@@ -71,6 +71,8 @@
     const b2_run* runs;
     const uint32_t* run_tile_base;
     const uint4* tile_info;
+    const uint32_t* group_heads;
+    TileRec* head_recs;
     TileRec* tiles;
     uint32_t* tile_base;
     uint32_t* tile_scratch;
@@ -96,6 +98,7 @@
     const DevMethod* methods;
     const uint32_t* crc_adv;
     uint32_t n_runs, n_tiles, max_msgs, max_resp;
+    uint32_t n_groups, walk_group;
 };
 
 template <bool kSpec, typename Emit>
@@ -224,42 +227,88 @@
     HdrWords h; h.w0 = __ldg(q); h.w1 = __ldg(q + 1); h.w2 = __ldg(q + 2); h.w3 = __ldg(q + 3);
     return h;
 }
+struct SpecAhead { HdrWords pre; uint32_t pre_pos, prev_len; };
+__device__ __forceinline__ Step spec_step(const uint8_t* run, uint32_t len, uint32_t pos, int pf, uint32_t ahead_end,
+                                          uint64_t max_body, bool client, uint32_t mask, SpecAhead& a) {
+    Step s;
+    bool fast = false;
+    if (len - pos >= 12) {
+        const HdrWords h = a.pre_pos == pos ? a.pre : load_hdr_words(run + pos);
+        const uint32_t guess = pos + a.prev_len;
+        if (a.prev_len && guess < ahead_end && (uint64_t)guess + 12 <= len) { a.pre = load_hdr_words(run + guess); a.pre_pos = guess; }
+        else a.pre_pos = kNone;
+        const uint32_t sh = 8u * (pos & 3u);
+        const uint32_t h0 = sh ? __funnelshift_r(h.w0, h.w1, sh) : h.w0, h1 = sh ? __funnelshift_r(h.w1, h.w2, sh) : h.w1,
+                       h2 = sh ? __funnelshift_r(h.w2, h.w3, sh) : h.w2;
+        const int idx = h0 == kMagicPRPC ? 1 : h0 == kMagicSTRM ? 2 : 0;
+        const uint32_t body = __byte_perm(h1, 0, 0x0123), meta = __byte_perm(h2, 0, 0x0123);
+        if (idx && ((mask >> idx) & 1u) && pf != 12 && (uint64_t)body <= max_body && (uint64_t)(len - pos) >= 12ull + body && meta <= body) {
+            s.err = B2_PARSE_OK; s.index = idx; s.pf = idx; s.frame_pos = pos; s.new_pos = pos + 12 + body; s.body = body; s.meta = meta; s.popped = false;
+            fast = true;
+        }
+    }
+    if (!fast) s = cut_input_message(run, len, pos, pf, max_body, client, mask);
+    return s;
+}
 template <typename Emit>
 __device__ __forceinline__ void walk_tile_spec(const uint8_t* run, uint32_t len, uint32_t entry, uint32_t tile_end,
                                                uint64_t max_body, bool client, TileRec& t, Emit emit, uint32_t mask) {
-    uint32_t pos = entry, count = 0, prev_len = 0, pre_pos = kNone;
+    uint32_t pos = entry, count = 0;
     int pf = -1, last = 0;
     uint8_t kind = kRanOff;
-    HdrWords pre; pre.w0 = pre.w1 = pre.w2 = pre.w3 = 0;
+    SpecAhead a; a.pre.w0 = a.pre.w1 = a.pre.w2 = a.pre.w3 = 0; a.pre_pos = kNone; a.prev_len = 0;
     while (pos < tile_end) {
-        Step s;
-        bool fast = false;
-        if (len - pos >= 12) {
-            const HdrWords h = pre_pos == pos ? pre : load_hdr_words(run + pos);
-            const uint32_t guess = pos + prev_len;
-            if (prev_len && guess < tile_end && (uint64_t)guess + 12 <= len) { pre = load_hdr_words(run + guess); pre_pos = guess; }
-            else pre_pos = kNone;
-            const uint32_t sh = 8u * (pos & 3u);
-            const uint32_t h0 = sh ? __funnelshift_r(h.w0, h.w1, sh) : h.w0, h1 = sh ? __funnelshift_r(h.w1, h.w2, sh) : h.w1,
-                           h2 = sh ? __funnelshift_r(h.w2, h.w3, sh) : h.w2;
-            const int idx = h0 == kMagicPRPC ? 1 : h0 == kMagicSTRM ? 2 : 0;
-            const uint32_t body = __byte_perm(h1, 0, 0x0123), meta = __byte_perm(h2, 0, 0x0123);
-            if (idx && ((mask >> idx) & 1u) && pf != 12 && (uint64_t)body <= max_body && (uint64_t)(len - pos) >= 12ull + body && meta <= body) {
-                s.err = B2_PARSE_OK; s.index = idx; s.pf = idx; s.frame_pos = pos; s.new_pos = pos + 12 + body; s.body = body; s.meta = meta; s.popped = false;
-                fast = true;
-            }
-        }
-        if (!fast) s = cut_input_message(run, len, pos, pf, max_body, client, mask);
+        const Step s = spec_step(run, len, pos, pf, tile_end, max_body, client, mask, a);
         if (count == 0 && (s.popped || (s.index != 12 && nshead_claims(run, len, pos, max_body, mask)))) { kind = kAmbig; break; }
         if (s.err != B2_PARSE_OK) { kind = kStop; break; }
         emit(count, s);
-        count++; last = s.index; pf = s.index; prev_len = s.new_pos - pos; pos = s.new_pos;
+        count++; last = s.index; pf = s.index; a.prev_len = s.new_pos - pos; pos = s.new_pos;
     }
     t.entry = entry; t.exit = pos; t.count = count; t.kind = kind; t.last_proto = (int8_t)last;
 }
 
-__global__ void __launch_bounds__(128) k_tile_walk(BatchPtrs B, DevConfig C) {
+__device__ __forceinline__ void walk_group_spec(const BatchPtrs& B, const DevConfig& C, uint32_t g) {
+    const uint32_t t0 = __ldg(B.group_heads + g);
+    const uint4 ti = __ldg(B.tile_info + t0);
+    const uint32_t k0 = ti.z, len = ti.y, flags = ti.w >> 24;
+    const uint8_t* run = B.bytes + ti.x;
+    const bool client = (flags & B2_RUN_CLIENT) != 0;
+    const uint32_t mask = run_mask(C.proto_mask, flags);
+    const uint32_t run_tiles = (uint32_t)(((uint64_t)len + C.tile_bytes - 1) >> C.tile_shift);
+    const uint32_t gn = min(B.walk_group, run_tiles - k0), group_end = (k0 + gn) << C.tile_shift;
+    uint32_t pos = B.head_recs[g].entry;
+    SpecAhead a; a.pre.w0 = a.pre.w1 = a.pre.w2 = a.pre.w3 = 0; a.pre_pos = kNone; a.prev_len = 0;
+    for (uint32_t m = 0; m < gn; m++) {
+        TileRec rec;
+        rec.entry = kNone; rec.exit = 0; rec.count = 0; rec.kind = kStop; rec.last_proto = 0; rec.live = 0; rec.pf_in = -1;
+        const uint32_t tile_end = (k0 + m + 1) << C.tile_shift;
+        if (pos < tile_end) {
+            uint32_t* spec = B.tile_spec + (size_t)(t0 + m) * C.spec_k;
+            uint32_t count = 0;
+            int pf = -1, last = 0;
+            uint8_t kind = kRanOff;
+            rec.entry = pos;
+            while (pos < tile_end) {
+                const Step s = spec_step(run, len, pos, pf, group_end, C.max_body_size, client, mask, a);
+                if (count == 0 && (s.popped || (s.index != 12 && nshead_claims(run, len, pos, C.max_body_size, mask)))) { kind = kAmbig; break; }
+                if (s.err != B2_PARSE_OK) { kind = kStop; break; }
+                if (count < C.spec_k) spec[count] = (ti.x + s.frame_pos) | ((uint32_t)(s.index != 1) << 31);
+                count++; last = s.index; pf = s.index; a.prev_len = s.new_pos - pos; pos = s.new_pos;
+            }
+            rec.exit = pos; rec.count = count; rec.kind = kind; rec.last_proto = (int8_t)last;
+            if (kind != kRanOff) pos = kNone;
+        }
+        B.tiles[t0 + m] = rec;
+    }
+}
+
+constexpr uint32_t kWalkGroupThreads = 64;
+__global__ void __launch_bounds__(128, 12) k_tile_walk(BatchPtrs B, DevConfig C) {
     const uint32_t t = blockIdx.x * blockDim.x + threadIdx.x;
+    if (B.walk_group > 1) {
+        if (t < B.n_groups) walk_group_spec(B, C, t);
+        return;
+    }
     if (t >= B.n_tiles) return;
     const uint4 ti = __ldg(B.tile_info + t);
     const uint32_t k = ti.z;
diff --git a/include/b2rpc.h b/include/b2rpc.h
--- a/include/b2rpc.h
+++ b/include/b2rpc.h
@@ -211,6 +211,9 @@
 int  b2_elapsed_ms(b2_ctx* a, b2_ctx* b, float* ms);
 
 int  b2_batch_info(b2_ctx* ctx, uint32_t out[4]);
+
+int  b2_set_walk_group(b2_ctx* ctx, uint32_t mode);
+int  b2_walk_group(b2_ctx* ctx);
 
 typedef struct b2_resident_kernel {
     const char* name;
```

After: 1.124 billion (median of 6 runs). 4.5% higher.
